# wardvdnb/Multimodal-SSL-AVMNIST

Hardware: NVIDIA B200
Metric: DINO train samples/sec (higher is better)
Workload: dtype bf16

## Files before the change

include/avmnist_b200.h:

```cpp
#ifndef AVMNIST_B200_H
#define AVMNIST_B200_H

#include <stdint.h>

#ifdef __cplusplus
extern "C" {
#endif

#define B200_E_ARG (-1)
#define B200_E_SHAPE (-2)
#define B200_E_SMEM (-3)

const char* b200_last_error(void);
int b200_abi_version(void);
int b200_device_sm_count(int device);
int b200_graph_node_counts(void* graph, int64_t* counts);

int b200_ema_flat(float* teacher, const float* student, int64_t n, float m, float one_minus_m, void* stream);
int b200_ema_multi(float* const* t_ptrs, const float* const* s_ptrs, const int64_t* offsets, int n_tensors,
                   int64_t total, float m, float one_minus_m, void* stream);

int b200_dino_loss_parts(int B);
int b200_dino_loss_fwd_bwd(const float* s, const float* t, const float* center, const float* t_colmean,
                           int Vs, int Vt, int B, int D, float tau_s, float tau_t, float grad_scale, int variant,
                           float* grad_s, float* part_loss, float* part_colsum, void* stream);
int b200_teacher_norm_colmean(const float* t, const float* center, int Vt, int B, int D, float* out, void* stream);

int b200_center_update(float* center, const float* part_colsum, const float* part_loss, int n_parts, int D,
                       int64_t n_rows, float m_c, float one_minus_mc, float* loss_out, float* colsum_out, void* stream);
int b200_center_apply(float* center, const float* colsum, int D, int64_t n_rows, float m_c, float one_minus_mc,
                      void* stream);

int64_t b200_loss_work_floats(int B);
int b200_mse_align_fwd_bwd(const float* a, const float* b, int B, int D, float grad_scale, float* grad_a,
                           float* grad_b, float* loss_out, float* work, void* stream);
int b200_ce_fwd_bwd(const float* logits, const int64_t* labels, int B, int C, float grad_scale, float* grad_logits,
                    float* loss_out, float* work, void* stream);
int64_t b200_infonce_work_floats(int B, int D);
int b200_infonce_fwd_bwd(const float* a, const float* b, int B, int D, float temperature, float grad_scale,
                         float* grad_a, float* grad_b, float* loss_out, float* work, void* stream);
int64_t b200_infonce_tc_work_floats(int B, int D);
int b200_infonce_fwd_bwd_tc(const float* a, const float* b, int B, int D, float temperature, float grad_scale, float* grad_a,
                            float* grad_b, float* loss_out, float* work, void* stream);
int64_t b200_ntxent_work_floats(int N, int D);
int b200_ntxent_fwd_bwd(const float* reps, int N, int D, float temperature, float grad_scale, float* grad, float* loss_out,
                        float* work, void* stream);
int b200_cosine_consistency_fwd_bwd(const float* emb, int V, int B, int D, float grad_scale, float* grad_emb,
                                    float* loss_out, float* work, void* stream);

#define B200_AUG_MAX_OPS 8
#define B200_AUG_GROUP_WORDS 28

int b200_aug_apply_image(const void* src, int src_u8, const int32_t* ops, float* out, void* out_quad8, int pad, int B,
                         int V, void* stream);
int b200_aug_apply_image_ex(const void* src, int src_u8, const int32_t* ops, const float* elastic_grid, uint64_t seed,
                            float* out, void* out_quad8, int pad, int B, int V, void* stream);
int b200_aug_apply_audio(const void* src, int src_u8, const int32_t* ops, const uint32_t* group_bits,
                         const float* noise, uint64_t seed, float* out, void* out_quad8, int pad, int B, int V,
                         void* stream);
int b200_aug_sample(const int32_t* spec, int B, int Vg, int Vl, uint64_t seed, uint64_t step, int32_t* img_ops,
                    int32_t* aud_ops, uint32_t* group_bits, void* stream);
int b200_aug_sample_dev(const int32_t* spec, int B, int Vg, int Vl, uint64_t seed, uint64_t step, const int64_t* step_dev,
                        int32_t* img_ops, int32_t* aud_ops, uint32_t* group_bits, void* stream);
int b200_aug_apply_audio_dev(const void* src, int src_u8, const int32_t* ops, const uint32_t* group_bits,
                             const float* noise, uint64_t seed, const int64_t* step_dev, float* out, void* out_quad8,
                             int pad, int B, int V, void* stream);

int b200_conv_supported(int Cin, int Cout, int H, int W, int K, int pad);
int b200_conv_fwd(const float* x, const float* w, const float* bias, float* z, double* stats, int N,
                  int n_per_view, int Cin, int Cout, int H, int W, int K, int pad, void* stream);
int b200_conv_bwd_data(const float* dz, const float* w, float* dx, int N, int Cin, int Cout, int H, int W, int K,
                       int pad, void* stream);
int b200_conv_tc_supported(int Cin, int Cout, int H, int W, int K, int pad);
int64_t b200_conv_tc_weight_bytes(int Cin, int Cout, int K);
int b200_conv_tc_prep_weights(const float* w, void* wprep, int Cin, int Cout, int K, int flip, void* stream);
int b200_conv_tc_prep_weights_multi(const int64_t* desc_dev, int n, void* stream);
int b200_conv_tc(const void* x_act8, const void* wprep, const float* bias, void* out, double* stats, int N,
                 int n_per_view, int Cin, int Cout, int H, int W, int K, int pad, int out_bf16, void* stream);
int b200_conv_tc_wgrad_variant(int tap);
int64_t b200_conv_tc_wgrad_work_floats(int N, int Cin, int Cout, int H, int W, int K, int pad);
int b200_conv_tc_wgrad(const void* x_act8, const void* dz_act8, float* dw, float* work, int N, int Cin, int Cout, int H,
                       int W, int K, int pad, void* stream);
int b200_pack_shift8(const float* x, void* out, int N, int H, int W, int pad, void* stream);
int b200_pack_quad8(const float* x, void* out, int N, int H, int W, int pad, void* stream);
int64_t b200_conv_tc_wgrad_l0_fused_work_floats(int N, int n_per_view, int Cout, int H, int W, int K, int pad);
int b200_conv_tc_wgrad_l0_fused(const void* x_quad8, const void* z8, const void* dp8, const float* scale, const float* shift,
                                const float* mean, const float* invstd, const double* sums, float* dw, double* dbsum,
                                float* work, int N, int n_per_view, int Cout, int H, int W, int K, int pad, void* stream);
int b200_conv_tc_pool_supported(int Cin, int Cout, int H, int W, int K, int pad);
int b200_conv_tc_pool(const void* x_act8, const void* wprep, const float* bias, const float* gamma, void* z_out, void* pool_out,
                      double* stats, int N, int n_per_view, int Cin, int Cout, int H, int W, int K, int pad, int z_fmt,
                      void* stream);
int b200_conv_tc_dgrad_bnstat_supported(int Cin, int Cout, int H, int W, int K, int pad);
int b200_conv_tc_dgrad_bnstat(const void* dz_act8, const void* wprep_flip, void* dx_act8, const void* p_act8, const float* gamma,
                              const float* beta, double* sums, int N, int n_per_view, int Cin, int Cout, int H, int W, int K,
                              int pad, void* stream);
int b200_bn_relu_apply8(const void* e8, const float* scale, const float* shift, void* out, int N, int n_per_view, int C, int HP,
                        int WP, int out_fmt, void* stream);
int b200_bn_relu_pool8_fwd(const void* z8, const float* scale, const float* shift, void* out, int N, int n_per_view,
                           int C, int H, int W, int z_f16, int out_fmt, void* stream);
int b200_bn_relu_pool8_bwd_reduce(const void* z8, const void* dp, const float* scale, const float* shift,
                                  const float* mean, const float* invstd, double* sums, int N, int n_per_view, int C,
                                  int H, int W, int z_f16, int dp_fmt, void* stream);
int b200_bn_relu_pool8_bwd_apply(const void* z8, const void* dp, const float* scale, const float* shift,
                                 const float* mean, const float* invstd, const double* sums, void* dz8, double* dbsum,
                                 int N, int n_per_view, int C, int H, int W, int z_f16, int dp_fmt, void* stream);
int b200_bn_pool8_bwd_reduce_p(const void* p, const void* dp, const float* gamma, const float* beta, double* sums, int N,
                               int n_per_view, int C, int HP, int WP, int p_fmt, int dp_fmt, void* stream);
int b200_bias_grad_finalize(const double* dbsum, float* db, int C, void* stream);
int b200_unpack_act8(const void* x8, float* out, int N, int C, int H, int W, void* stream);
int b200_pack_act8(const float* x, void* out, int N, int C, int H, int W, void* stream);
int64_t b200_conv_bwd_weight_work_floats(int N, int Cin, int Cout, int H, int W, int K, int pad);
int b200_conv_bwd_weight(const float* x, const float* dz, float* dw, float* db, float* work, int N, int Cin,
                         int Cout, int H, int W, int K, int pad, void* stream);

int b200_bn_finalize(const double* stats, const float* gamma, const float* beta, float* running_mean,
                     float* running_var, int64_t* num_batches_tracked, float* scale, float* shift, float* mean,
                     float* invstd, int n_views, int C, int64_t count, float momentum, float eps, int train,
                     void* stream);
int b200_bn_relu_pool_fwd(const float* z, const float* scale, const float* shift, float* out, int N,
                          int n_per_view, int C, int H, int W, void* stream);
int b200_bn_relu_pool_bwd_reduce(const float* z, const float* dout, const float* scale, const float* shift,
                                 const float* mean, const float* invstd, double* sums, int N, int n_per_view,
                                 int C, int H, int W, void* stream);
int b200_bn_relu_pool_bwd_apply(const float* z, const float* dout, const float* scale, const float* shift,
                                const float* mean, const float* invstd, const double* sums, float* dz, int N,
                                int n_per_view, int C, int H, int W, void* stream);
int b200_bn_param_grads(const double* sums, float* dgamma, float* dbeta, int n_views, int C, int accumulate,
                        void* stream);
int b200_avgpool_fwd(const float* x, float* out, int N, int C, int HW, void* stream);
int b200_avgpool_bwd(const float* dout, float* dx, int N, int C, int HW, void* stream);

int b200_linear_fwd(const float* x, int64_t ldx, const float* w, const float* bias, float* y, int64_t ldy, int M,
                    int N, int K, int act, const uint8_t* mask, float drop_p, void* stream);
int b200_linear_bwd_data(const float* dy, int64_t lddy, const float* w, float* dx, int64_t lddx, int M, int N,
                         int K, void* stream);
int64_t b200_linear_bwd_weight_work_floats(int M, int N, int K);
int b200_linear_bwd_weight(const float* dy, int64_t lddy, const float* x, int64_t ldx, float* dw, float* db, float* work,
                           int M, int N, int K, int accumulate, void* stream);
int b200_linear_fwd_tc(const float* x, int64_t ldx, const float* w, const float* bias, float* y, int64_t ldy, int M, int N,
                       int K, int act, const uint8_t* mask, float drop_p, void* stream);
int64_t b200_linear_bwd_data_tc_work_floats(int M, int N, int K);
int b200_linear_bwd_data_tc(const float* dy, int64_t lddy, const float* w, float* dx, int64_t lddx, float* work, int M, int N,
                            int K, void* stream);
int64_t b200_linear_bwd_weight_tc_work_floats(int M, int N, int K);
int b200_linear_bwd_weight_tc(const float* dy, int64_t lddy, const float* x, int64_t ldx, float* dw, float* db, float* work,
                              int M, int N, int K, int accumulate, void* stream);
int b200_act_bwd(float* dy, const float* y, const uint8_t* mask, float drop_p, int64_t n, void* stream);
int b200_colstats(const float* h, double* stats, int M, int C, void* stream);
int b200_bn1d_gelu_drop_fwd(const float* h, const float* scale, const float* shift, const uint8_t* mask,
                            float drop_p, float* g, int M, int C, void* stream);
int b200_bn1d_gelu_drop_bwd_reduce(const float* h, const float* dg, const float* scale, const float* shift,
                                   const float* mean, const float* invstd, const uint8_t* mask, float drop_p,
                                   double* sums, int M, int C, void* stream);
int b200_bn1d_gelu_drop_bwd_apply(const float* h, const float* dg, const float* scale, const float* shift,
                                  const float* mean, const float* invstd, const uint8_t* mask, float drop_p,
                                  const double* sums, float* dh, int M, int C, void* stream);
int b200_dropout_mask(uint8_t* mask, int64_t n, float p, uint64_t seed, uint64_t offset, void* stream);
int b200_dropout_mask_dev(uint8_t* mask, int64_t n, float p, uint64_t seed, uint64_t offset, const int64_t* step_dev,
                          void* stream);

int b200_adam_flat(float* param, const float* grad, float* exp_avg, float* exp_avg_sq, int64_t n, float lr,
                   float beta1, float beta2, float eps, float weight_decay, float bias_correction1,
                   float bias_correction2_sqrt, float grad_scale, void* stream);
int b200_adam_bias_dev(const int64_t* step_dev, double beta1, double beta2, float* bc_out, void* stream);
int b200_adam_flat_dev(float* param, const float* grad, float* exp_avg, float* exp_avg_sq, int64_t n, float lr,
                       float beta1, float beta2, float eps, float weight_decay, const float* bc_dev, float grad_scale,
                       void* stream);
int b200_counters_advance(int64_t* counters, int n, void* stream);
int b200_scale_flat(float* y, int64_t n, float alpha, void* stream);

int b200_knn_neg_half_sqnorm(const float* x, int64_t ldx, int N, int D, float* out, void* stream);
int b200_knn_topk_vote(const float* scores, int64_t lds, const int64_t* labels, int M, int N, int k, int n_classes,
                       int64_t* pred, int32_t* neighbours, void* stream);

int b200_gate_apply(const float* x, int64_t ldx, float* y, int64_t ldy, const float* gate, int M, int N, void* stream);
int64_t b200_gate_grad_work_floats(void);
int b200_gate_grad(const float* dy, int64_t lddy, const float* x, int64_t ldx, const float* gate, float* dgate, float* work, int M, int N,
                   int accumulate, void* stream);
int b200_softmax_rows(float* s, int64_t ld, int M, int N, float scale, void* stream);
int b200_softmax_rows_bwd(float* dp, int64_t lddp, const float* p, int64_t ldp, int M, int N, float scale, void* stream);
int b200_add2d(float* dst, int64_t ld_dst, const float* src, int64_t ld_src, int M, int N, void* stream);

int b200_dp_nccl_version(void);
int b200_dp_unique_id(char* id_out );
int b200_dp_init(const char* id , int rank, int world);
int b200_dp_world(void);
int b200_dp_rank(void);
int b200_dp_allreduce_grads(float* grad, int64_t n, void* stream);
int b200_dp_allreduce_center(float* colsum, int D, void* stream);
int b200_dp_destroy(void);

#ifdef __cplusplus
}
#endif
#endif
```

multimodal_ssl_avmnist_b200/contrastive.py:

```python
import math

import numpy as np
import torch

from . import dp
from . import ops
from .engine import F32, Arena, DinoStepEngine, _BN, _conv, _lin, _vec2, head_params

IMG_LAYERS = [("image_encoder.encoder.0", "image_encoder.encoder.1", 1, 32, 28, 3, 1), ("image_encoder.encoder.4", "image_encoder.encoder.5", 32, 64, 14, 3, 1),
              ("image_encoder.encoder.8", "image_encoder.encoder.9", 64, 128, 7, 3, 1)]
AUD_LAYERS = [("audio_encoder.encoder.0", "audio_encoder.encoder.1", 1, 32, 112, 3, 1), ("audio_encoder.encoder.4", "audio_encoder.encoder.5", 32, 64, 56, 3, 1),
              ("audio_encoder.encoder.8", "audio_encoder.encoder.9", 64, 128, 28, 3, 1), ("audio_encoder.encoder.12", "audio_encoder.encoder.13", 128, 256, 14, 3, 1)]
MODES = (("img", "img"), ("aud", "aud"), ("img", "aud"), ("aud", "img"))


def contrastive_params(O, P):
    img = []
    for i, (ci, co) in zip((0, 4, 8), ((1, 32), (32, 64), (64, 128))):
        img += _conv(f"image_encoder.encoder.{i}", co, ci, 3) + _vec2(f"image_encoder.encoder.{i + 1}", co)
    img += _lin("image_encoder.encoder.14", 512, 128) + _lin("image_encoder.projection.0", O, 512)
    img += [("image_projection_head." + n, s) for n, s in head_params(O, P)]
    aud = []
    for i, (ci, co) in zip((0, 4, 8, 12), ((1, 32), (32, 64), (64, 128), (128, 256))):
        aud += _conv(f"audio_encoder.encoder.{i}", co, ci, 3) + _vec2(f"audio_encoder.encoder.{i + 1}", co)
    aud += _lin("audio_encoder.encoder.18", O, 256)
    aud += [("audio_projection_head." + n, s) for n, s in head_params(O, P)]
    return img, aud


class ContrastiveStepEngine(DinoStepEngine):
    def __init__(self, kind="infonce", output_dim=256, projection_dim=256, learning_rate=1e-4, temperature=0.07, seed=0, device=None,
                 precision="bf16", fused_pool=False, process_group=None, data_parallel=None, mode_seed=0):
        if not torch.cuda.is_available():
            raise ops._lib.B200Error("ContrastiveStepEngine needs a CUDA device: the hot path has no CPU fallback")
        ops._lib.load()
        assert kind in ("infonce", "simclr") and precision in ("bf16", "fp32")
        self.device = torch.device(device if device is not None else f"cuda:{torch.cuda.current_device()}")
        self.kind, self.mode, self.precision = kind, "default", precision
        self.lin_tc = precision == "bf16"
        self.multi, self.mix = False, None
        self.O, self.P = output_dim, projection_dim
        self.lr, self.weight_decay, self.temperature = learning_rate, 0.0, temperature
        self.seed, self.rng_step = seed, 0
        self.pg = process_group
        self.world = dp.world_size(process_group) if (data_parallel is None or data_parallel) else 1
        self.comm, self._comm_stream = None, None
        self._ctr = self._bc = self._graph = None
        self.img_layers, self.aud_layers = IMG_LAYERS, AUD_LAYERS
        img, aud = contrastive_params(self.O, self.P)
        self.student = Arena([("enc." + n, s) for n, s in img + aud], self.device)
        self.branch_range = {"img": self.student.range_of(["enc." + n for n, _ in img]), "aud": self.student.range_of(["enc." + n for n, _ in aud])}
        self.step_counts = {"img": 0, "aud": 0}
        self.grad = torch.zeros_like(self.student.flat)
        self.exp_avg, self.exp_avg_sq = torch.zeros_like(self.student.flat), torch.zeros_like(self.student.flat)
        self.S, self.G = self.student.views(), self.student.views(self.grad)
        self.bn_s = {}
        for conv, bn, ci, co, hw, k, pad in IMG_LAYERS + AUD_LAYERS:
            self.bn_s["enc." + bn] = _BN(co, self.device)
        for m in ("image", "audio"):
            self.bn_s[f"enc.{m}_projection_head.mlp.1"] = _BN(512, self.device)
        self.tc = {}
        for mod, layers in (("img", IMG_LAYERS), ("aud", AUD_LAYERS)):
            self.tc[mod] = [precision == "bf16" and ops.conv_tc_supported(ci, co, hw, hw, k, pad) and
                            (ci == 1 or ops.conv_tc_supported(co, ci, hw + 2 * pad - k + 1, hw + 2 * pad - k + 1, k, k - 1 - pad))
                            for (conv, bn, ci, co, hw, k, pad) in layers]
        self.fused_pool = bool(fused_pool)
        self.pool = {"s": {mod: [self.fused_pool and bool(self.tc[mod][li]) and ops.conv_tc_pool_supported(ci, co, hw, hw, k, pad) and ci == 1 and hw >= 112
                                 for li, (conv, bn, ci, co, hw, k, pad) in enumerate(layers)] for mod, layers in (("img", IMG_LAYERS), ("aud", AUD_LAYERS))}}
        self.pool["t"] = self.pool["s"]
        self.fused_bnstat = False
        self.bnstat = {mod: [False] * len(layers) for mod, layers in (("img", IMG_LAYERS), ("aud", AUD_LAYERS))}
        self._tcw, self._prep_desc = {}, {}
        for mod, layers in (("img", IMG_LAYERS), ("aud", AUD_LAYERS)):
            for li, (conv, bn, ci, co, hw, k, pad) in enumerate(layers):
                if self.tc[mod][li]:
                    self._tcw[("s", mod, li)] = torch.empty(ops.conv_tc_weight_bytes(ci, co, k), dtype=torch.uint8, device=self.device)
                    if ci > 1:
                        self._tcw[("flip", mod, li)] = torch.empty(ops.conv_tc_weight_bytes(co, ci, k), dtype=torch.uint8, device=self.device)
        self.overlap_teacher = True
        self.stream_priorities, self._main_stream = False, None
        self._side_stream = torch.cuda.Stream(device=self.device)
        self._lin_wg_stream = torch.cuda.Stream(device=self.device)
        self._lin_wg_pending = False
        self._wgrad_streams = {m: torch.cuda.Stream(device=self.device) for m in ("img", "aud")}
        self._eval_wrole = "s"
        self._ws = {}
        self._mode_rng = torch.Generator().manual_seed(mode_seed)
        if self.world > 1:
            self.comm = dp.AbiComm.get(process_group)
            self._comm_stream = torch.cuda.Stream(device=self.device)
        self._comm_pending = False
        self._init_parameters()

    def _init_parameters(self):
        g = torch.Generator(device="cpu").manual_seed(self.seed)
        bn_bases = set(self.bn_s)
        bounds = {}
        for name, shape in self.student.spec:
            v = self.student.view(name)
            base = name.rsplit(".", 1)[0]
            if base in bn_bases:
                v.fill_(1.0 if name.endswith(".weight") else 0.0)
            else:
                if len(shape) > 1:
                    bounds[base] = 1.0 / math.sqrt(int(np.prod(shape[1:])))
                v.copy_(((torch.rand(shape, generator=g) * 2 - 1) * bounds[base]).to(self.device))

    def load_named(self, params):
        for m, d in params.items():
            for k, v in d.items():
                self.S[f"enc.{m}.{k}"].copy_(v.to(self.device))

    def sync_teacher(self):
        pass

    def _dino_only(self, *a, **k):
        raise ops._lib.B200Error("this entry point belongs to the DINO step engine; the contrastive engine offers forward_backward / "
                                 "optimizer_step / train_step_views / train_step / capture_train_step / graph_step")

    forward_pass = dino_loss_pass = aux_loss_pass = backward_pass = update_teacher = train_step_host = encode_features = begin_probe = _dino_only
    augment = augment_with_params = prefetch_augment = allreduce_gradients = graph_node_counts = _dino_only

    def _workspace(self, B):
        if B in self._ws:
            return self._ws[B]
        dev, BF = self.device, torch.bfloat16

        def e(*shape, dtype=F32):
            return torch.empty(*shape, dtype=dtype, device=dev)

        w = {"B": B}
        zarena = torch.zeros(1 << 16, dtype=torch.float64, device=dev)
        zoff = [0]

        def zalloc(*shape):
            n = int(math.prod(shape))
            o = zoff[0]
            zoff[0] = o + (n + 1) // 2 * 2
            if zoff[0] > zarena.numel():
                raise ops._lib.B200Error("zero arena too small")
            return zarena[o:o + n].view(*shape)

        w["zarena"] = zarena
        N = 2 * B
        w["x_img"], w["x_aud"] = e(N, 1, 28, 28), e(N, 1, 112, 112)
        for mod, layers in (("img", IMG_LAYERS), ("aud", AUD_LAYERS)):
            sc = dict(wg=0, z=0, p=0, z8=0)
            for li, (conv, bn, ci, co, hw, k, pad) in enumerate(layers):
                ho = hw + 2 * pad - k + 1
                tc = self.tc[mod][li]
                next_tc = li + 1 < len(layers) and self.tc[mod][li + 1]
                if tc and ci == 1:
                    w[f"{mod}.xs8"] = e(N, hw, ops.quad8_width(hw, pad), 8, dtype=BF)
                if tc and self.pool["s"][mod][li]:
                    w[f"s.{mod}.e{li}"] = e(N, co // 8, ho // 2, ho // 2, 8, dtype=torch.float16)
                w[f"s.{mod}.z{li}"] = e(N, co // 8, ho, ho, 8, dtype=torch.float16) if tc else e(N, co, ho, ho)
                if next_tc:
                    w[f"s.{mod}.p8{li}"] = e(N, co // 8, ho // 2, ho // 2, 8, dtype=BF)
                if not next_tc or not tc:
                    w[f"s.{mod}.p{li}"] = e(N, co, ho // 2, ho // 2)
                w[f"s.{mod}.stats{li}"] = zalloc(2, co, 2)
                w[f"s.{mod}.sums{li}"] = zalloc(2, co, 2)
                for nm in ("scale", "shift", "mean", "invstd"):
                    w[f"s.{mod}.{nm}{li}"] = e(2, co)
                if tc:
                    sc["wg"] = max(sc["wg"], ops.conv_tc_wgrad_work_floats(N, ci, co, hw, hw, k, pad))
                    if ci == 1:
                        sc["wg"] = max(sc["wg"], ops.conv_tc_wgrad_l0_fused_work_floats(N, B, co, hw, hw, k, pad))
                    else:
                        sc["z8"] = max(sc["z8"], N * co * ho * ho)
                else:
                    sc["wg"] = max(sc["wg"], ops.conv_bwd_weight_work_floats(N, ci, co, hw, hw, k, pad))
                    sc["z"] = max(sc["z"], N * co * ho * ho)
                sc["p"] = max(sc["p"], N * co * (ho // 2) * (ho // 2), N * ci * hw * hw if li > 0 else 0)
            w[f"{mod}.dz"] = e(max(sc["z"], 4))
            w[f"{mod}.dz8"] = e(max(sc["z8"], 8), dtype=BF)
            w[f"{mod}.dz8b"] = e(max(sc["z8"], 8), dtype=BF)
            w[f"{mod}.dbsum"] = zalloc(8, 256)
            w[f"{mod}.dp_a"], w[f"{mod}.dp_b"] = e(sc["p"]), e(sc["p"])
            w[f"{mod}.wg_work"], w[f"{mod}.wg_work_b"] = e(max(sc["wg"], 4)), e(max(sc["wg"], 4))
        O, P = self.O, self.P
        w["img.gap"], w["img.e14"], w["aud.gap"] = e(N, 128), e(N, 512), e(N, 256)
        w["d.img.gap"], w["d.img.e14"], w["d.aud.gap"] = e(N, 128), e(N, 512), e(N, 256)
        for mod in ("img", "aud"):
            w[f"{mod}.feat"], w[f"d.{mod}.feat"] = e(N, O), e(N, O)
            w[f"{mod}.hh"], w[f"{mod}.g"], w[f"{mod}.d.hh"], w[f"{mod}.d.g"] = e(N, 512), e(N, 512), e(N, 512), e(N, 512)
            w[f"{mod}.hstats"], w[f"{mod}.hsums"] = zalloc(2, 512, 2), zalloc(2, 512, 2)
            for nm in ("hscale", "hshift", "hmean", "hinvstd"):
                w[f"{mod}.{nm}"] = e(2, 512)
        w["reps"], w["d.reps"] = e(N, P), e(N, P)
        w["loss"] = torch.zeros(4, device=dev)
        w["ntxent_work"] = e(ops.ntxent_work_floats(N, P))
        w["infonce_work"] = e(ops.infonce_work_floats(B, P, tc=self.lin_tc))
        self._ws[B] = w
        return w

    def _combo(self, w, mod, calls):
        key = ("combo", mod, calls)
        if key in w:
            return w[key]
        B = w["B"]
        N = calls * B
        c = {"B": B, "zarena": w["zarena"], "packed": False}
        for k, v in w.items():
            if not isinstance(k, str) or not isinstance(v, torch.Tensor):
                continue
            if k.startswith(f"s.{mod}.") and k.split(".")[2].rstrip("0123456789") in ("stats", "sums", "scale", "shift", "mean", "invstd"):
                c[k] = v[:calls]
            elif k.startswith(f"s.{mod}.") or k == f"{mod}.xs8":
                c[k] = v[:N]
            elif k.startswith(f"{mod}."):
                c[k] = v
        w[key] = c
        return c

    def _branch_fwd(self, w, mod, x, calls):
        B, S = w["B"], self.S
        N = calls * B
        c = self._combo(w, mod, calls)
        layers = IMG_LAYERS if mod == "img" else AUD_LAYERS
        hw = layers[0][4]
        xin = w[f"x_{mod}"][:N]
        xin.copy_(x.reshape(N, 1, hw, hw))
        if self.tc[mod][0]:
# ... 231 lines not shown
```

multimodal_ssl_avmnist_b200/csrc/conv_tc.cu:

```cuda
#include <cuda_bf16.h>

#include "common.cuh"
#include "umma.cuh"

namespace b200 {

int encode_tmap_bf16_4d(CUtensorMap* out, const void* base, const uint64_t dims[4], const uint64_t strides_bytes[3],
                        const uint32_t box[4]) {
    typedef CUresult (*EncodeFn)(CUtensorMap*, CUtensorMapDataType, cuuint32_t, void*, const cuuint64_t*, const cuuint64_t*,
                                 const cuuint32_t*, const cuuint32_t*, CUtensorMapInterleave, CUtensorMapSwizzle,
                                 CUtensorMapL2promotion, CUtensorMapFloatOOBfill);
    static EncodeFn fn = nullptr;
    if (!fn) {
        void* p = nullptr;
        cudaDriverEntryPointQueryResult q;
        cudaError_t e = cudaGetDriverEntryPoint("cuTensorMapEncodeTiled", &p, cudaEnableDefault, &q);
        if (e != cudaSuccess || q != cudaDriverEntryPointSuccess || !p) {
            set_error("cuTensorMapEncodeTiled entry point not available (%d)", (int)e);
            return -30;
        }
        fn = (EncodeFn)p;
    }
    cuuint64_t d[4] = {dims[0], dims[1], dims[2], dims[3]};
    cuuint64_t s[3] = {strides_bytes[0], strides_bytes[1], strides_bytes[2]};
    cuuint32_t b[4] = {box[0], box[1], box[2], box[3]};
    cuuint32_t es[4] = {1, 1, 1, 1};
    CUresult r = fn(out, CU_TENSOR_MAP_DATA_TYPE_BFLOAT16, 4, const_cast<void*>(base), d, s, b, es, CU_TENSOR_MAP_INTERLEAVE_NONE,
                    CU_TENSOR_MAP_SWIZZLE_NONE, CU_TENSOR_MAP_L2_PROMOTION_L2_128B, CU_TENSOR_MAP_FLOAT_OOB_FILL_NONE);
    if (r != CUDA_SUCCESS) {
        set_error("cuTensorMapEncodeTiled failed (%d)", (int)r);
        return -31;
    }
    return 0;
}

namespace {

using namespace umma;

constexpr int round_up(int a, int b) { return (a + b - 1) / b * b; }
constexpr int SMEM_EST(int nmma, int npad, int slots, int slot_bytes, int tail) { return round_up(nmma * npad * 32, 128) + slots * slot_bytes + tail + 256 + npad * 4; }
constexpr int nbuf_for(int npadl, int ctas) {
    int n = (npadl <= 32 ? 8 : 4) / (ctas > 2 ? 2 : 1);
    while (n > 1 && n * npadl * ctas > 512) n /= 2;
    return n;
}
constexpr int pow2_cols(int c) { return c <= 32 ? 32 : c <= 64 ? 64 : c <= 128 ? 128 : c <= 256 ? 256 : 512; }

__host__ __device__ constexpr int xph_for(int cin, int cout, int ks) {
    return (ks == 5 && ((cin == 8 && cout == 16) || (cin == 16 && cout == 8))) ? 4
         : (ks == 5 && ((cin == 16 && cout == 32) || (cin == 32 && cout == 16))) ? 2
         : (ks == 3 && ((cin == 32 && cout == 64) || (cin == 64 && cout == 32))) ? 2 : 1;
}

struct TMaps {
    CUtensorMap m[4];
};

constexpr int nbuf_chunked(int tiles, int npadl, int ctas) {
    int m = 512 / (ctas * npadl * tiles);
    while (m > 1 && m * tiles > 8) --m;
    return (m < 1 ? 1 : m) * tiles;
}

template <int CIN_, int COUT_, int NPAD_, int HIN_, int WIN_, int KS_, int PAD_, int BANDS_, int SLOTS_, int CTAS_ = 1, int NSPLIT_ = 1, int KCH_ = 1>
struct TcCfg {
    static constexpr int NSPLIT = NSPLIT_;
    static constexpr int KCH = KCH_;
    static constexpr int XPH = CIN_ == 1 ? 4 : xph_for(CIN_, COUT_, KS_);
    static constexpr int XPL = CIN_ == 1 ? 1 : XPH;
    __host__ __device__ static constexpr int col_phase(int col) { return (col / 8) % XPH; }
    __host__ __device__ static constexpr int col_channel(int col) { return (col / 8) / XPH * 8 + col % 8; }
    static constexpr int NPADL = XPH == 1 ? NPAD_ / NSPLIT_ : round_up(XPH * COUT_, 16), COUTL = COUT_ / NSPLIT_;
    static_assert(NSPLIT_ == 1 || (XPH == 1 && COUT_ == NPAD_ && NPADL % 16 == 0), "N split needs C_out == NPAD and 16-channel slices");
    static constexpr int CIN = CIN_, COUT = COUT_, NPAD = NPAD_, HIN = HIN_, WIN = WIN_, KS = KS_, PAD = PAD_, BANDS = BANDS_, SLOTS = SLOTS_;
    static constexpr int CTAS = CTAS_;
    static constexpr bool L0 = (CIN == 1);
    static constexpr int P = L0 ? 1 : CIN / 8;
    static constexpr int WP = WIN + 2 * PAD;
    static constexpr int HO = HIN + 2 * PAD - KS + 1, WO = WP - KS + 1;
    static constexpr int HB = HO / BANDS;
    static constexpr int HPB = HB + KS - 1;
    static constexpr int KWX = KS + XPH - 1;
    static constexpr int WQ = (WP + XPH - 1) / XPH;
    static constexpr int WOQ = WO / XPH;
    static constexpr int Q = (HB - 1) * WQ + WOQ;
    static constexpr int TILES = (Q + 127) / 128;
    static constexpr int PLANE_BYTES = HPB * WQ * 16;
    static constexpr int PC = P / KCH;
    static constexpr int PHASE_BYTES = round_up(PC * PLANE_BYTES, 128);
    static constexpr int SLOT_BYTES = round_up(XPL * PHASE_BYTES, 128);
    static constexpr int NJ = (KWX + 1) / 2;
    static constexpr int PH = P / 2;
    static constexpr int PHC = PC / 2;
    static constexpr int NMMA = L0 ? (KS + 1) / 2 : (CIN == 8) ? KS * NJ : KS * KWX * PH;
    static constexpr int W_BYTES = round_up(NMMA * NPADL * 32, 128);
    static constexpr int MAXPIX = TILES * 128 + (L0 ? KS : KS - 1) * WQ + (KWX - 1) / XPH + 2;
    static constexpr int TAIL = round_up((MAXPIX > HPB * WQ ? (MAXPIX - HPB * WQ) : 0) * 16, 128) + 128;
    static_assert(XPH == 1 || (WO % XPH == 0 && WIN % XPH == 0 && XPH <= 4 && (CIN != 8 || (XPH % 2 == 0 && KWX % 2 == 0))), "x phases");
    static_assert(!L0 || KWX <= 8, "first layer: all taps of all phases must lie inside one 8-pixel unit");
    static constexpr int IMG_BYTES = SLOTS * SLOT_BYTES + TAIL;
    static constexpr int BAR_OFF = W_BYTES + IMG_BYTES;
    static constexpr bool POOL_OK = (CIN_ == 1 || COUT_ > CIN_) && NSPLIT_ == 1 && HO % 2 == 0 && HB % 2 == 0 && WO % 2 == 0 && XPH % 2 == 0;
    static constexpr bool BSTAT_OK = CIN_ > COUT_ && NSPLIT_ == 1;
    static constexpr int POOL_R = 128 / WQ + 3;
    static constexpr int OCTL = COUTL / 8;
    static constexpr int POOL_ROW_UNITS = (WO / 2) * OCTL;
    static constexpr int POOL_BYTES = POOL_OK ? POOL_R * POOL_ROW_UNITS * 16 : 0;
    static constexpr int SIGN_OFF = BAR_OFF + 256 + NPADL * 4;
    static constexpr int POOL_OFF = round_up(SIGN_OFF + NPADL * 2, 16);
    static constexpr int SMEM = POOL_OFF + POOL_BYTES;
    static constexpr int SMEM_NOPOOL = SIGN_OFF + NPADL * 4;
    static constexpr int NBUF = KCH > 1 ? nbuf_chunked(TILES, NPADL, CTAS) : nbuf_for(NPADL, CTAS);
    static_assert(KCH == 1 || (CIN >= 16 && P % KCH == 0 && PC % 2 == 0 && NBUF % TILES == 0 && NBUF * NPADL * CTAS <= 512), "K chunking");
    static constexpr int TMEM_COLS = pow2_cols(NBUF * NPADL);
    static constexpr int ISS = CTAS >= 3 ? 1 : (CTAS == 2 ? 2 : 4);
    static constexpr int THREADS = 32 * (1 + ISS + 4);
    static_assert(TILES % ISS == 0 || NBUF % TILES == 0, "a TMEM stage must always be filled by the same issuer");
    static_assert(KCH > 1 || NBUF % ISS == 0, "a TMEM stage must always be filled by the same issuer");
    static_assert(TMEM_COLS * CTAS <= 512, "TMEM columns per SM");
    static_assert((SMEM_EST(NMMA, NPADL, SLOTS, SLOT_BYTES, TAIL) + POOL_BYTES + NPADL * 2 + 16 + 1024) * CTAS <= 227 * 1024, "shared memory per SM");
    static_assert(2 * SLOTS + 2 * NBUF <= 24, "barrier area");
    static_assert(CIN == 1 || (CIN % 8 == 0 && (CIN == 8 || CIN % 16 == 0)), "C_in must be 1, 8 or a multiple of 16");
    static_assert(NPAD % 16 == 0 && NPAD >= 16 && NPADL <= 128 && COUT <= NPAD && COUT % 8 == 0, "N tile");
    static_assert(HO % BANDS == 0, "bands must divide the output height");
    static_assert(SMEM <= 227 * 1024, "shared memory budget");
    static_assert(XPL * PHASE_BYTES < (1 << 18) && PLANE_BYTES % 16 == 0, "descriptor range");
};

__device__ __forceinline__ void ld_global_nc_256(const uint4* p, uint4& a, uint4& b) {
    asm volatile("ld.global.nc.v8.b32 {%0, %1, %2, %3, %4, %5, %6, %7}, [%8];"
                 : "=r"(a.x), "=r"(a.y), "=r"(a.z), "=r"(a.w), "=r"(b.x), "=r"(b.y), "=r"(b.z), "=r"(b.w)
                 : "l"(p));
}
__device__ __forceinline__ uint32_t hmax2_u32(uint32_t a, uint32_t b) {
    uint32_t d;
    asm("max.f16x2 %0, %1, %2;" : "=r"(d) : "r"(a), "r"(b));
    return d;
}
template <class C>
__device__ __forceinline__ int pool_unit(int h, int xq) {
    if constexpr (C::XPH % 2 == 0) {
        const int col0 = h * 16;
        if (col0 >= C::XPH * C::COUTL) return -1;
        const int ph0 = C::col_phase(col0), oct0 = C::col_channel(col0) / 8;
        return ((xq * C::XPH + ph0) >> 1) * C::OCTL + oct0;
    } else {
        const int oct = h;
        if (oct * 8 >= C::COUTL) return -1;
        return (xq >> 1) * C::OCTL + oct;
    }
}

template <class C, bool POOL, bool BSTAT = false>
__global__ void __launch_bounds__(C::THREADS, C::CTAS)
conv_tc_kernel(const __grid_constant__ TMaps tmaps, const uint4* __restrict__ wprep, const float* __restrict__ bias,
               void* __restrict__ out, double* __restrict__ stats, int n_per_view, int out_bf16,
               uint4* __restrict__ pool_out, const float* __restrict__ gamma, const float* __restrict__ beta2 = nullptr) {
    extern __shared__ __align__(1024) uint8_t smem[];
    uint8_t* w_s = smem;
    uint8_t* img_s = smem + C::W_BYTES;
    uint64_t* bars = reinterpret_cast<uint64_t*>(smem + C::BAR_OFF);
    uint32_t* tmem_slot = reinterpret_cast<uint32_t*>(smem + C::BAR_OFF + 200);
    float* bias_s = reinterpret_cast<float*>(smem + C::BAR_OFF + 256);
    uint32_t* sign_s = reinterpret_cast<uint32_t*>(smem + C::SIGN_OFF);
    float* ig_s = reinterpret_cast<float*>(smem + C::SIGN_OFF);
    uint4* stash = reinterpret_cast<uint4*>(smem + C::POOL_OFF);

    const int warp = threadIdx.x >> 5, lane = threadIdx.x & 31;
    const int view = blockIdx.y, G = gridDim.x, g = blockIdx.x;
    const long items = (long)n_per_view * C::BANDS;
    const int i0 = (int)(items * g / G), i1 = (int)(items * (g + 1) / G);

    const uint32_t bar0 = smem_u32(bars);
    auto full_bar = [&](int s) { return bar0 + 8u * s; };
    auto empty_bar = [&](int s) { return bar0 + 8u * (C::SLOTS + s); };
    auto tfull_bar = [&](int b) { return bar0 + 8u * (2 * C::SLOTS + b); };
    auto tempty_bar = [&](int b) { return bar0 + 8u * (2 * C::SLOTS + C::NBUF + b); };

    {
        const uint4* src = wprep;
        uint4* dst = reinterpret_cast<uint4*>(w_s);
        constexpr int NGL = C::NPADL / 8, NG = NGL * C::NSPLIT;
        for (int i = threadIdx.x; i < C::NMMA * 2 * NGL * 8; i += blockDim.x) {
            const int q = i & 7, gl = (i >> 3) % NGL, mc = (i >> 3) / NGL;
            dst[i] = src[(mc * NG + blockIdx.z * NGL + gl) * 8 + q];
        }
        uint4* z = reinterpret_cast<uint4*>(img_s);
        for (int i = threadIdx.x; i < C::IMG_BYTES / 16; i += blockDim.x) z[i] = make_uint4(0, 0, 0, 0);
        for (int i = threadIdx.x; i < C::NPADL; i += blockDim.x)
            bias_s[i] = (bias != nullptr && i < C::XPH * C::COUTL) ? bias[blockIdx.z * C::COUTL + C::col_channel(i)] : 0.f;
        if constexpr (BSTAT) {
            for (int i = threadIdx.x; i < C::NPADL; i += blockDim.x) {
                const bool real = i < C::XPH * C::COUTL;
                const float gm = real ? gamma[blockIdx.z * C::COUTL + C::col_channel(i)] : 0.f;
                ig_s[i] = gm != 0.f ? 1.0f / gm : 0.f;
                bias_s[i] = real ? beta2[blockIdx.z * C::COUTL + C::col_channel(i)] : 0.f;
            }
        }
        if constexpr (POOL) {
            for (int i = threadIdx.x; i < C::NPADL / 2; i += blockDim.x) {
                uint32_t m = 0;
#pragma unroll
                for (int h = 0; h < 2; ++h) {
                    const int col = 2 * i + h;
                    if (gamma != nullptr && col < C::XPH * C::COUTL && gamma[blockIdx.z * C::COUTL + C::col_channel(col)] < 0.f) m |= 0x8000u << (16 * h);
                }
                sign_s[i] = m;
            }
        }
        fence_proxy_async_smem();
    }
    if (warp == 0 && lane == 0) {
        for (int r = 0; r < C::XPL; ++r) prefetch_tmap(&tmaps.m[r]);
        for (int s = 0; s < C::SLOTS; ++s) {
            mbar_init(full_bar(s), 1);
            mbar_init(empty_bar(s), C::ISS);
        }
        for (int b = 0; b < C::NBUF; ++b) {
            mbar_init(tfull_bar(b), 1);
            mbar_init(tempty_bar(b), 4);
        }
        fence_mbar_init();
    }
    if (warp == 1) tmem_alloc<C::TMEM_COLS>(smem_u32(tmem_slot));
    tc_fence_before_sync();
    __syncthreads();
    tc_fence_after_sync();
    const uint32_t tmem_base = *tmem_slot;
    const uint32_t img_addr = smem_u32(img_s), w_addr = smem_u32(w_s);

    if (warp == 0) {
        if (lane == 0) {
            for (int i = i0; i < i1; ++i) {
                const int n = view * n_per_view + i / C::BANDS, band = i % C::BANDS;
#pragma unroll 1
                for (int c = 0; c < C::KCH; ++c) {
                    const int k = (i - i0) * C::KCH + c, slot = k % C::SLOTS, use = k / C::SLOTS;
                    mbar_wait(empty_bar(slot), (use & 1) ^ 1);
                    mbar_expect_tx(full_bar(slot), C::XPL * C::PC * C::PLANE_BYTES);
#pragma unroll
                    for (int rp = 0; rp < C::XPL; ++rp) {
                        constexpr int X = C::XPH;
                        const int r = ((rp - C::PAD) % X + X) % X, a = (rp - C::PAD - r) / X;
                        tma_load_4d(img_addr + slot * C::SLOT_BYTES + rp * C::PHASE_BYTES, &tmaps.m[r], full_bar(slot), 0, C::L0 ? 0 : a,
                                    band * C::HB - C::PAD, n * C::P + c * C::PC);
                    }
                }
            }
        }
    } else if (warp <= C::ISS) {
        if (lane == 0) {
            constexpr uint32_t idesc = idesc_bf16(C::NPADL);
            for (int i = i0; i < i1; ++i) {
#pragma unroll 1
              for (int c = 0; c < C::KCH; ++c) {
                const int k = (i - i0) * C::KCH + c, slot = k % C::SLOTS, use = k / C::SLOTS;
                mbar_wait(full_bar(slot), use & 1);
                tc_fence_after_sync();
                const uint32_t slot_addr = img_addr + slot * C::SLOT_BYTES;
                for (int t = warp - 1; t < C::TILES; t += C::ISS) {
                    const uint32_t tcount = (uint32_t)(i - i0) * C::TILES + t;
                    const uint32_t buf = tcount % C::NBUF, u = tcount / C::NBUF;
                    if (c == 0) {
                        mbar_wait(tempty_bar(buf), (u & 1) ^ 1);
                        tc_fence_after_sync();
                    }
                    const uint32_t d = tmem_base + buf * C::NPADL;
                    const uint32_t a0 = slot_addr + t * 2048;
                    int idx = 0;
                    if constexpr (C::L0) {
#pragma unroll
                        for (int j = 0; j < C::NMMA; ++j, ++idx) {
                            const uint64_t ad = smem_desc(a0 + (2 * j * C::WQ) * 16, C::WQ * 16, 128);
                            const uint64_t bd = smem_desc(w_addr + idx * C::NPADL * 32, C::NPADL * 16, 128);
                            mma_bf16(d, ad, bd, idesc, idx > 0);
                        }
                    } else {
#pragma unroll
                    for (int kh = 0; kh < C::KS; ++kh) {
                        if constexpr (C::CIN == 8) {
#pragma unroll
                            for (int j = 0; j < C::NJ; ++j, ++idx) {
                                const uint64_t ad = smem_desc(a0 + ((2 * j) % C::XPH) * C::PHASE_BYTES + (kh * C::WQ + (2 * j) / C::XPH) * 16,
                                                              C::XPH == 1 ? 16 : C::PHASE_BYTES, 128);
                                const uint64_t bd = smem_desc(w_addr + idx * C::NPADL * 32, C::NPADL * 16, 128);
                                mma_bf16(d, ad, bd, idesc, idx > 0);
                            }
                        } else {
#pragma unroll
                            for (int kw = 0; kw < C::KWX; ++kw) {
#pragma unroll
                                for (int pp = 0; pp < C::PHC; ++pp, ++idx) {
                                    const int widx = (kh * C::KWX + kw) * C::PH + c * C::PHC + pp;
                                    const uint64_t ad = smem_desc(a0 + (kw % C::XPH) * C::PHASE_BYTES + (kh * C::WQ + kw / C::XPH) * 16 +
                                                                      pp * 2 * C::PLANE_BYTES, C::PLANE_BYTES, 128);
                                    const uint64_t bd = smem_desc(w_addr + widx * C::NPADL * 32, C::NPADL * 16, 128);
                                    mma_bf16(d, ad, bd, idesc, (c > 0 || idx > 0) ? 1u : 0u);
                                }
                            }
                        }
                    }
                    }
                    if (c == C::KCH - 1) mma_commit(tfull_bar(buf));
                }
                mma_commit(empty_bar(slot));
              }
            }
        }
    } else {
        const int quad = warp & 3, row = quad * 32 + lane;
        float s1[C::COUTL], s2[C::COUTL];
#pragma unroll
        for (int c = 0; c < C::COUTL; ++c) s1[c] = s2[c] = 0.f;
        const int co0 = blockIdx.z * C::COUTL;
        const bool do_stats = BSTAT ? (stats != nullptr) : ((bias != nullptr) && (stats != nullptr));
        constexpr int NCH = C::NPADL / 16;
        constexpr int NHP = POOL ? (C::XPH % 2 == 0 ? NCH : 2 * NCH) : 1;
        uint32_t tcount = 0;
        for (int i = i0; i < i1; ++i) {
            const int n = view * n_per_view + i / C::BANDS, band = i % C::BANDS;
            for (int t = 0; t < C::TILES; ++t, ++tcount) {
                [[maybe_unused]] uint4 hp[NHP];
                const uint32_t buf = tcount % C::NBUF, u = tcount / C::NBUF;
                const int q = t * 128 + row;
                const int y = q / C::WQ, xq = q - y * C::WQ;
                const bool valid = (y < C::HB) && (xq < C::WOQ);
                const int yy = band * C::HB + y;
                [[maybe_unused]] uint4 ppre[BSTAT ? NCH : 1][2];
                if constexpr (BSTAT) {
#pragma unroll
                    for (int cc = 0; cc < NCH; ++cc) {
                        const int col0 = cc * 16;
                        ppre[cc][0] = ppre[cc][1] = make_uint4(0, 0, 0, 0);
                        if (valid && col0 < C::XPH * C::COUTL) {
                            const int ph0 = C::col_phase(col0), oct0 = C::col_channel(col0) / 8;
                            const uint4* pin = pool_out;
                            if constexpr (C::XPH % 2 == 0) {
                                ld_global_nc_256(pin + (((long)n * (C::COUT / 8) + co0 / 8 + oct0) * C::HO + yy) * C::WO + xq * C::XPH + ph0, ppre[cc][0],
                                                 ppre[cc][1]);
                            } else {
                                ppre[cc][0] = __ldg(pin + (((long)n * (C::COUT / 8) + co0 / 8 + oct0) * C::HO + yy) * C::WO + xq);
                                if ((oct0 + 1) * 8 < C::COUTL)
                                    ppre[cc][1] = __ldg(pin + (((long)n * (C::COUT / 8) + co0 / 8 + oct0 + 1) * C::HO + yy) * C::WO + xq);
                            }
                        }
                    }
                }
                mbar_wait(tfull_bar(buf), u & 1);
                tc_fence_after_sync();
                const uint32_t taddr = tmem_base + ((uint32_t)(quad * 32) << 16) + buf * C::NPADL;
#pragma unroll
                for (int cc = 0; cc < C::NPADL / 16; ++cc) {
                    uint32_t v[16];
                    tmem_ld16(taddr + cc * 16, v);
                    tmem_ld_wait();
                    if (cc == C::NPADL / 16 - 1) {
                        tc_fence_before_sync();
                        __syncwarp();
                        if (lane == 0) mbar_arrive(tempty_bar(buf));
                    }
                    float f[16];
#pragma unroll
                    for (int j = 0; j < 16; ++j) {
                        const int col = cc * 16 + j, ch = C::col_channel(col);
                        if constexpr (BSTAT) {
                            f[j] = __uint_as_float(v[j]);
                        } else {
                            f[j] = __uint_as_float(v[j]) + bias_s[col];
                            if (col < C::XPH * C::COUTL && valid) {
                                s1[ch] += f[j];
                                s2[ch] += f[j] * f[j];
                            }
                        }
                    }
                    if constexpr (BSTAT) {
                        const int col0 = cc * 16;
                        if (valid && col0 < C::XPH * C::COUTL) {
                            const uint4 pa = ppre[cc][0], pb = ppre[cc][1];
                            const uint32_t pw[8] = {pa.x, pa.y, pa.z, pa.w, pb.x, pb.y, pb.z, pb.w};
#pragma unroll
                            for (int j = 0; j < 16; ++j) {
                                const int col = col0 + j, ch = C::col_channel(col);
                                const float pv = __uint_as_float((j & 1) ? (pw[j >> 1] & 0xFFFF0000u) : (pw[j >> 1] << 16));
                                const float gr = __bfloat162float(__float2bfloat16_rn(f[j]));
                                if (col < C::XPH * C::COUTL && pv > 0.f) {
                                    s1[ch] += gr;
                                    s2[ch] += gr * ((pv - bias_s[col]) * ig_s[col]);
                                }
                            }
                        }
                    }
                    if constexpr (POOL) {
                        {
                            uint4 a, b;
                            a.x = pack_f16(f[0], f[1]); a.y = pack_f16(f[2], f[3]); a.z = pack_f16(f[4], f[5]); a.w = pack_f16(f[6], f[7]);
                            b.x = pack_f16(f[8], f[9]); b.y = pack_f16(f[10], f[11]); b.z = pack_f16(f[12], f[13]); b.w = pack_f16(f[14], f[15]);
                            const uint4 ma = *reinterpret_cast<const uint4*>(sign_s + cc * 8), mb = *reinterpret_cast<const uint4*>(sign_s + cc * 8 + 4);
                            a.x ^= ma.x; a.y ^= ma.y; a.z ^= ma.z; a.w ^= ma.w;
                            b.x ^= mb.x; b.y ^= mb.y; b.z ^= mb.z; b.w ^= mb.w;
                            if constexpr (C::XPH % 2 == 0) {
                                hp[cc].x = hmax2_u32(a.x, b.x); hp[cc].y = hmax2_u32(a.y, b.y); hp[cc].z = hmax2_u32(a.z, b.z); hp[cc].w = hmax2_u32(a.w, b.w);
                            } else {
                                hp[2 * cc].x = hmax2_u32(a.x, __shfl_xor_sync(0xffffffffu, a.x, 1)); hp[2 * cc].y = hmax2_u32(a.y, __shfl_xor_sync(0xffffffffu, a.y, 1));
                                hp[2 * cc].z = hmax2_u32(a.z, __shfl_xor_sync(0xffffffffu, a.z, 1)); hp[2 * cc].w = hmax2_u32(a.w, __shfl_xor_sync(0xffffffffu, a.w, 1));
                                hp[2 * cc + 1].x = hmax2_u32(b.x, __shfl_xor_sync(0xffffffffu, b.x, 1)); hp[2 * cc + 1].y = hmax2_u32(b.y, __shfl_xor_sync(0xffffffffu, b.y, 1));
                                hp[2 * cc + 1].z = hmax2_u32(b.z, __shfl_xor_sync(0xffffffffu, b.z, 1)); hp[2 * cc + 1].w = hmax2_u32(b.w, __shfl_xor_sync(0xffffffffu, b.w, 1));
                            }
                        }
                    }
                    if (valid && (!POOL || out != nullptr)) {
                        if (out_bf16) {
                            uint4 pk[2];
#pragma unroll
                            for (int o = 0; o < 2; ++o) {
                                if (out_bf16 == 2) {
                                    pk[o].x = pack_f16(f[o * 8 + 0], f[o * 8 + 1]);
                                    pk[o].y = pack_f16(f[o * 8 + 2], f[o * 8 + 3]);
                                    pk[o].z = pack_f16(f[o * 8 + 4], f[o * 8 + 5]);
                                    pk[o].w = pack_f16(f[o * 8 + 6], f[o * 8 + 7]);
                                } else {
                                    pk[o].x = pack_bf16(f[o * 8 + 0], f[o * 8 + 1]);
                                    pk[o].y = pack_bf16(f[o * 8 + 2], f[o * 8 + 3]);
                                    pk[o].z = pack_bf16(f[o * 8 + 4], f[o * 8 + 5]);
                                    pk[o].w = pack_bf16(f[o * 8 + 6], f[o * 8 + 7]);
                                }
                            }
                            const int col0 = cc * 16, ph0 = C::col_phase(col0), oct0 = C::col_channel(col0) / 8;
                            if constexpr (C::XPH % 2 == 0) {
                                if (col0 < C::XPH * C::COUTL) {
                                    uint4* dst = reinterpret_cast<uint4*>(out) + (((long)n * (C::COUT / 8) + co0 / 8 + oct0) * C::HO + yy) * C::WO +
                                                 xq * C::XPH + ph0;
                                    st_global_256(dst, pk[0], pk[1]);
                                }
                            } else {
#pragma unroll
                                for (int o = 0; o < 2; ++o) {
                                    const int oct = oct0 + o;
                                    if (oct * 8 < C::COUTL) {
                                        uint4* dst = reinterpret_cast<uint4*>(out) + (((long)n * (C::COUT / 8) + co0 / 8 + oct) * C::HO + yy) * C::WO + xq;
                                        *dst = pk[o];
                                    }
                                }
                            }
                        } else {
                            float* dst = reinterpret_cast<float*>(out) + (((long)n * C::COUT + co0) * C::HO + yy) * C::WO + xq * C::XPH;
#pragma unroll
                            for (int j = 0; j < 16; ++j) {
                                const int col = cc * 16 + j, ph = C::col_phase(col), ch = C::col_channel(col);
                                if (col < C::XPH * C::COUTL) dst[(long)ch * C::HO * C::WO + ph] = f[j];
                            }
                        }
                    }
                }
                if constexpr (POOL) {
                    {
                        const int slot = (int)(((long)(i - i0) * (C::HB / 2) + (y >> 1)) % C::POOL_R);
                        const bool own = valid && (C::XPH % 2 == 0 || (xq & 1) == 0);
                        uint4* srow = stash + slot * C::POOL_ROW_UNITS;
                        if (own && (y & 1) == 0) {
#pragma unroll
                            for (int h = 0; h < NHP; ++h) {
                                const int u = pool_unit<C>(h, xq);
                                if (u >= 0) srow[u] = hp[h];
                            }
                        }
                        asm volatile("bar.sync 2, 128;" ::: "memory");
                        if (own && (y & 1) == 1) {
                            const int ypg = (band * C::HB + y) >> 1;
                            uint4 ev[NHP];
#pragma unroll
                            for (int h = 0; h < NHP; ++h) {
                                const int u = pool_unit<C>(h, xq);
                                if (u >= 0) {
                                    const uint4 up = srow[u];
                                    const int col0 = (C::XPH % 2 == 0 ? h : h / 2) * 16 + (C::XPH % 2 == 0 ? 0 : (h & 1) * 8);
                                    const uint4 m = *reinterpret_cast<const uint4*>(sign_s + col0 / 2);
                                    ev[h].x = hmax2_u32(hp[h].x, up.x) ^ m.x; ev[h].y = hmax2_u32(hp[h].y, up.y) ^ m.y;
                                    ev[h].z = hmax2_u32(hp[h].z, up.z) ^ m.z; ev[h].w = hmax2_u32(hp[h].w, up.w) ^ m.w;
                                }
                            }
                            const long plane = (long)(C::HO / 2) * (C::WO / 2);
                            uint4* erow = pool_out + ((long)n * (C::COUT / 8) + co0 / 8) * plane + (long)ypg * (C::WO / 2);
                            if constexpr (C::XPH == 4) {
#pragma unroll
                                for (int h = 0; h + 1 < NHP; h += 2) {
                                    const int u = pool_unit<C>(h, xq);
                                    if (u >= 0) {
                                        const int xp = u / C::OCTL, oct = u - xp * C::OCTL;
                                        st_global_256(erow + oct * plane + xp, ev[h], ev[h + 1]);
                                    }
                                }
                            } else {
#pragma unroll
                                for (int h = 0; h < NHP; ++h) {
                                    const int u = pool_unit<C>(h, xq);
                                    if (u >= 0) {
                                        const int xp = u / C::OCTL, oct = u - xp * C::OCTL;
                                        erow[oct * plane + xp] = ev[h];
                                    }
                                }
                            }
                        }
                    }
                }
            }
        }
        if (do_stats) {
#pragma unroll
            for (int c = 0; c < C::COUTL; ++c) {
                const double a = warp_sum((double)s1[c]), b = warp_sum((double)s2[c]);
                if (lane == 0) {
                    atomicAdd(&stats[((long)view * C::COUT + co0 + c) * 2 + 0], a);
                    atomicAdd(&stats[((long)view * C::COUT + co0 + c) * 2 + 1], b);
                }
            }
        }
    }
    tc_fence_before_sync();
    __syncthreads();
    if (warp == 1) {
        tc_fence_after_sync();
        tmem_dealloc<C::TMEM_COLS>(tmem_base);
    }
}

__device__ __forceinline__ void conv_tc_prep_element(const float* __restrict__ w, __nv_bfloat16* __restrict__ out, int CIN, int COUT, int NPAD,
                                                     int KS, int XPH, int flip, int e) {
    const int k8 = e & 7, r = (e >> 3) & 7, NG = NPAD / 8;
    const int ng = (e >> 6) % NG, c = (e / (64 * NG)) & 1, m = e / (128 * NG);
    const int ph = ng % XPH, co = ng / XPH * 8 + r;
    const int KWX = KS + XPH - 1;
    int kh, kw, ci;
    if (CIN == 1) {
        kh = 2 * m + c;
        kw = k8 - ph;
        ci = 0;
        float v1 = 0.f;
        if (kh < KS && kw >= 0 && kw < KS && co < COUT) v1 = w[(co * KS + kh) * KS + kw];
        out[e] = __float2bfloat16_rn(v1);
        return;
    } else if (CIN == 8) {
        const int NJ = (KWX + 1) / 2;
        kh = m / NJ;
        kw = 2 * (m % NJ) + c - ph;
        ci = k8;
    } else {
        const int PH = CIN / 16;
        kh = m / (KWX * PH);
        kw = (m / PH) % KWX - ph;
        ci = (2 * (m % PH) + c) * 8 + k8;
    }
    float v = 0.f;
    if (kw >= 0 && kw < KS && co < COUT) {
        v = flip ? w[((ci * COUT + co) * KS + (KS - 1 - kh)) * KS + (KS - 1 - kw)] : w[((co * CIN + ci) * KS + kh) * KS + kw];
    }
    out[e] = __float2bfloat16_rn(v);
}

__global__ void conv_tc_prep_weights_kernel(const float* __restrict__ w, __nv_bfloat16* __restrict__ out, int CIN, int COUT, int NPAD,
                                            int KS, int XPH, int flip, int total) {
    const int e = blockIdx.x * blockDim.x + threadIdx.x;
    if (e < total) conv_tc_prep_element(w, out, CIN, COUT, NPAD, KS, XPH, flip, e);
}

__host__ __device__ inline void conv_tc_weight_geometry(int Cin, int Cout, int K, int* xph, int* npad, int* total) {
    const int x = Cin == 1 ? 4 : xph_for(Cin, Cout, K), kwx = K + x - 1;
    const int np = (x * Cout + 15) / 16 * 16;
    const int nmma = (Cin == 1) ? (K + 1) / 2 : (Cin == 8) ? K * ((kwx + 1) / 2) : K * kwx * (Cin / 16);
    *xph = x;
    *npad = np;
    *total = nmma * np * 16;
}

__global__ void conv_tc_prep_weights_multi_kernel(const long long* __restrict__ desc) {
    const long long* d = desc + 6 * blockIdx.y;
    const int Cin = (int)d[2], Cout = (int)d[3], K = (int)d[4], flip = (int)d[5];
    int xph, npad, total;
    conv_tc_weight_geometry(Cin, Cout, K, &xph, &npad, &total);
    const float* w = reinterpret_cast<const float*>(d[0]);
    __nv_bfloat16* out = reinterpret_cast<__nv_bfloat16*>(d[1]);
    for (int e = blockIdx.x * blockDim.x + threadIdx.x; e < total; e += gridDim.x * blockDim.x)
        conv_tc_prep_element(w, out, Cin, Cout, npad, K, xph, flip, e);
}

__global__ void pack_act8_kernel(const float* __restrict__ x, uint4* __restrict__ out, long n_units, int C, int HW) {
    const long i = (long)blockIdx.x * blockDim.x + threadIdx.x;
    if (i >= n_units) return;
    const int pix = (int)(i % HW);
    const long no = i / HW;
    const int oct = (int)(no % (C / 8));
    const long n = no / (C / 8);
    const float* s = x + ((n * C + oct * 8) * (long)HW) + pix;
    uint4 pk;
    pk.x = pack_bf16(s[0], s[(long)HW]);
    pk.y = pack_bf16(s[2L * HW], s[3L * HW]);
    pk.z = pack_bf16(s[4L * HW], s[5L * HW]);
    pk.w = pack_bf16(s[6L * HW], s[7L * HW]);
    out[i] = pk;
}

__global__ void pack_shift8_kernel(const float* __restrict__ x, uint4* __restrict__ out, long n_units, int W, int pad) {
    const long i = (long)blockIdx.x * blockDim.x + threadIdx.x;
    if (i >= n_units) return;
    const int WT = W + pad;
    const int xs = (int)(i % WT);
    const long row = i / WT;
    const float* r = x + row * W;
    float f[8];
#pragma unroll
    for (int c = 0; c < 8; ++c) {
        const int xc = xs - pad + c;
        f[c] = (xc >= 0 && xc < W) ? __ldg(r + xc) : 0.f;
    }
    out[i] = make_uint4(pack_bf16(f[0], f[1]), pack_bf16(f[2], f[3]), pack_bf16(f[4], f[5]), pack_bf16(f[6], f[7]));
}

__global__ void pack_quad8_kernel(const float* __restrict__ x, uint4* __restrict__ out, long n_units, int W, int WQ, int pad) {
    const long i = (long)blockIdx.x * blockDim.x + threadIdx.x;
    if (i >= n_units) return;
    const int xq = (int)(i % WQ);
    const long row = i / WQ;
    const float* r = x + row * W;
    float f[8];
#pragma unroll
    for (int c = 0; c < 8; ++c) {
        const int xc = 4 * xq - pad + c;
        f[c] = (xc >= 0 && xc < W) ? __ldg(r + xc) : 0.f;
    }
    out[i] = make_uint4(pack_bf16(f[0], f[1]), pack_bf16(f[2], f[3]), pack_bf16(f[4], f[5]), pack_bf16(f[6], f[7]));
}

template <class C>
int launch_conv_tc(const void* x, const void* wprep, const float* bias, void* out, double* stats, int N, int n_per_view, int out_bf16,
                   cudaStream_t st, void* pool_out = nullptr, const float* gamma = nullptr, const float* beta2 = nullptr) {
    if (pool_out != nullptr && beta2 == nullptr && !C::POOL_OK) {
        set_error("conv_tc: this geometry has no fused max-pool epilogue");
        return -5;
    }
    static bool configured = false;
    if (!configured) {
        cudaError_t e = cudaFuncSetAttribute(conv_tc_kernel<C, false>, cudaFuncAttributeMaxDynamicSharedMemorySize, C::SMEM_NOPOOL);
        if (e == cudaSuccess && C::POOL_OK) e = cudaFuncSetAttribute(conv_tc_kernel<C, C::POOL_OK>, cudaFuncAttributeMaxDynamicSharedMemorySize, C::SMEM);
        if (e == cudaSuccess && C::BSTAT_OK)
            e = cudaFuncSetAttribute(conv_tc_kernel<C, false, C::BSTAT_OK>, cudaFuncAttributeMaxDynamicSharedMemorySize, C::SMEM_NOPOOL);
        if (e != cudaSuccess) {
            set_error("conv_tc: cannot set %d bytes of shared memory: %s", C::SMEM, cudaGetErrorString(e));
            return (int)e;
        }
        configured = true;
    }
    TMaps tm;
    constexpr uint64_t WT = C::L0 ? C::WQ : C::WIN;
    for (int r = 0; r < C::XPL; ++r) {
        const uint64_t dims[4] = {8, WT / C::XPL, (uint64_t)C::HIN, (uint64_t)N * C::P};
        const uint64_t strides[3] = {16 * (uint64_t)C::XPL, WT * 16, WT * C::HIN * 16};
        const uint32_t box[4] = {8, (uint32_t)C::WQ, (uint32_t)C::HPB, (uint32_t)C::PC};
        int rc = encode_tmap_bf16_4d(&tm.m[r], reinterpret_cast<const uint8_t*>(x) + 16 * r, dims, strides, box);
        if (rc) return rc;
    }
    for (int r = C::XPL; r < 4; ++r) tm.m[r] = tm.m[0];
    const int views = N / n_per_view;
    int G = sm_count() * C::CTAS / (views * C::NSPLIT);
    if (G < 1) G = 1;
    const long items = (long)n_per_view * C::BANDS;
    if (G > items) G = (int)items;
    if (beta2 != nullptr) {
        if (!C::BSTAT_OK) {
            set_error("conv_tc: this geometry has no fused BatchNorm-backward statistics");
            return -5;
        }
        conv_tc_kernel<C, false, C::BSTAT_OK><<<dim3(G, views, C::NSPLIT), C::THREADS, C::SMEM_NOPOOL, st>>>(
            tm, reinterpret_cast<const uint4*>(wprep), nullptr, out, stats, n_per_view, out_bf16, reinterpret_cast<uint4*>(pool_out), gamma, beta2);
    } else if (pool_out != nullptr)
        conv_tc_kernel<C, C::POOL_OK><<<dim3(G, views, C::NSPLIT), C::THREADS, C::SMEM, st>>>(tm, reinterpret_cast<const uint4*>(wprep), bias, out, stats,
                                                                                              n_per_view, out_bf16, reinterpret_cast<uint4*>(pool_out), gamma);
    else
        conv_tc_kernel<C, false><<<dim3(G, views, C::NSPLIT), C::THREADS, C::SMEM_NOPOOL, st>>>(tm, reinterpret_cast<const uint4*>(wprep), bias, out, stats,
                                                                                                n_per_view, out_bf16, nullptr, nullptr);
    return launch_status("conv_tc_kernel");
}

constexpr int hbz_for(int hb, int wp) {
    int h = hb;
    while ((h * wp) % 16) ++h;
    return h;
}

template <int CIN_, int COUT_, int HIN_, int WIN_, int KS_, int PAD_, int BANDS_, int SLOTS_, int PSPLIT_, int CTAS_ = 1, int NSPLIT_ = 1>
struct TcWgCfg {
    static constexpr int NSPLIT = NSPLIT_, COUTL = COUT_ / NSPLIT_;
    static constexpr int CTAS = CTAS_;
    static constexpr int CIN = CIN_, COUT = COUT_, HIN = HIN_, WIN = WIN_, KS = KS_, PAD = PAD_, BANDS = BANDS_, SLOTS = SLOTS_, PSPLIT = PSPLIT_;
    static constexpr bool L0 = (CIN == 1);
    static constexpr int P_IN = L0 ? 1 : CIN / 8, P_OUT = COUT / 8, P_OUTL = COUTL / 8, PI = P_IN / PSPLIT;
    static constexpr int WP = WIN + 2 * PAD;
    static constexpr int HO = HIN + 2 * PAD - KS + 1, WO = WP - KS + 1;
    static constexpr int HB = HO / BANDS, HPB = HB + KS - 1;
    static constexpr int HBZ = hbz_for(HB, WP);
    static constexpr int KSTEPS = HBZ * WP / 16;
    static constexpr int PLANE_X = HPB * WP * 16, PLANE_Z = HBZ * WP * 16;
    static constexpr int X_BYTES = round_up(PI * PLANE_X, 128), Z_BYTES = round_up(P_OUTL * PLANE_Z, 128);
    static constexpr int SLOT_BYTES = X_BYTES + Z_BYTES;
    static constexpr int NACC = L0 ? 1 : KS * PI;
    static constexpr int TMEM_COLS = pow2_cols(NACC * COUTL);
    static constexpr int ONES_OFF = SLOTS * SLOT_BYTES;
    static constexpr int BAR_OFF = ONES_OFF;
    static constexpr int SMEM = BAR_OFF + 256;
    static constexpr int DW = COUT * CIN * KS * KS;
    static constexpr int PART = DW;
    static_assert(P_IN % PSPLIT == 0 && HO % BANDS == 0, "splits");
    static_assert(BANDS == 1 || HBZ == HB, "row bands need HB*WP to be a multiple of 16");
    static constexpr int ISS = (L0 || NACC < 4 || CTAS >= 3) ? 1 : (NACC <= 6 ? NACC : 4);
    static constexpr int THREADS = 32 * (1 + ISS + 4);
    static_assert(NACC * COUTL <= 512 && TMEM_COLS * CTAS <= 512 && COUTL % 8 == 0, "TMEM columns");
    static_assert((SMEM + 1024) * CTAS <= 227 * 1024, "shared memory per SM");
    static_assert(KS <= 8 && COUT % 8 == 0 && COUT >= 8 && COUT <= 256, "shape");
    static_assert((KSTEPS * 16 + (L0 ? 7 : KS - 1) * WP + 8 - HPB * WP) * 16 <= Z_BYTES, "x overrun must stay inside the slot");
    static_assert(SMEM <= 227 * 1024, "shared memory budget");
};

template <class C>
__global__ void __launch_bounds__(C::THREADS, C::CTAS)
conv_tc_wgrad_kernel(const __grid_constant__ CUtensorMap tmap_x, const __grid_constant__ CUtensorMap tmap_z, float* __restrict__ work, int N) {
    extern __shared__ __align__(1024) uint8_t smem[];
    uint64_t* bars = reinterpret_cast<uint64_t*>(smem + C::BAR_OFF);
    uint32_t* tmem_slot = reinterpret_cast<uint32_t*>(smem + C::BAR_OFF + 192);
    const int warp = threadIdx.x >> 5, lane = threadIdx.x & 31;
    const int G = gridDim.x, g = blockIdx.x, split = blockIdx.z % C::PSPLIT, ns = blockIdx.z / C::PSPLIT;
    const long items = (long)N * C::BANDS;
    const int i0 = (int)(items * g / G), i1 = (int)(items * (g + 1) / G);
    const uint32_t bar0 = smem_u32(bars);
    auto full_bar = [&](int s) { return bar0 + 8u * s; };
    auto empty_bar = [&](int s) { return bar0 + 8u * (C::SLOTS + s); };
    const uint32_t done_bar = bar0 + 8u * (2 * C::SLOTS);
    {
        uint4* z = reinterpret_cast<uint4*>(smem);
        for (int i = threadIdx.x; i < C::ONES_OFF / 16; i += blockDim.x) z[i] = make_uint4(0, 0, 0, 0);
        fence_proxy_async_smem();
    }
    if (warp == 0 && lane == 0) {
        prefetch_tmap(&tmap_x);
        prefetch_tmap(&tmap_z);
        for (int s = 0; s < C::SLOTS; ++s) {
            mbar_init(full_bar(s), 1);
            mbar_init(empty_bar(s), C::ISS);
        }
        mbar_init(done_bar, C::ISS);
        fence_mbar_init();
    }
    if (warp == 1) tmem_alloc<C::TMEM_COLS>(smem_u32(tmem_slot));
    tc_fence_before_sync();
    __syncthreads();
    tc_fence_after_sync();
    const uint32_t tmem_base = *tmem_slot;
    const uint32_t smem0 = smem_u32(smem);

    if (warp == 0) {
        if (lane == 0) {
            for (int i = i0; i < i1; ++i) {
                const int k = i - i0, slot = k % C::SLOTS, use = k / C::SLOTS;
                mbar_wait(empty_bar(slot), (use & 1) ^ 1);
                mbar_expect_tx(full_bar(slot), C::PI * C::PLANE_X + C::P_OUTL * C::PLANE_Z);
                const int n = i / C::BANDS, band = i % C::BANDS;
                const uint32_t sa = smem0 + slot * C::SLOT_BYTES;
                tma_load_4d(sa, &tmap_x, full_bar(slot), 0, C::L0 ? 0 : -C::PAD, band * C::HB - C::PAD, n * C::P_IN + split * C::PI);
                tma_load_4d(sa + C::X_BYTES, &tmap_z, full_bar(slot), 0, 0, band * C::HB, n * C::P_OUT + ns * C::P_OUTL);
            }
        }
    } else if (warp <= C::ISS) {
        if (lane == 0) {
            constexpr uint32_t idesc = idesc_bf16(C::COUTL, true, true, 64);
            for (int i = i0; i < i1; ++i) {
                const int k = i - i0, slot = k % C::SLOTS, use = k / C::SLOTS;
                mbar_wait(full_bar(slot), use & 1);
                tc_fence_after_sync();
                const uint32_t xa = smem0 + slot * C::SLOT_BYTES, za = xa + C::X_BYTES;
                for (int ks = 0; ks < C::KSTEPS; ++ks) {
                    const uint32_t acc = (i > i0 || ks > 0) ? 1u : 0u;
                    const uint64_t bd = smem_desc(za + ks * 256, 128, C::PLANE_Z);
                    if constexpr (C::L0) {
                        const uint64_t ad = smem_desc(xa + ks * 256, 128, C::WP * 16);
                        mma_bf16(tmem_base, ad, bd, idesc, acc);
                    } else {
#pragma unroll
                        for (int kh = 0; kh < C::KS; ++kh) {
#pragma unroll
                            for (int pl = 0; pl < C::PI; ++pl) {
                                if ((kh * C::PI + pl) % C::ISS != warp - 1) continue;
                                const uint64_t ad = smem_desc(xa + pl * C::PLANE_X + (ks * 16 + kh * C::WP) * 16, 128, 16);
                                mma_bf16(tmem_base + (kh * C::PI + pl) * C::COUTL, ad, bd, idesc, acc);
                            }
                        }
                    }
                }
                mma_commit(empty_bar(slot));
            }
            mma_commit(done_bar);
        }
    } else {
        const int quad = warp & 3;
        const int m = quad * 16 + (lane & 15), j = m >> 3, ci8 = m & 7;
        const bool rowok = (lane < 16) && (j < C::KS);
        float* part = work + (long)g * C::PART;
        if (i1 > i0) {
            mbar_wait(done_bar, 0);
            tc_fence_after_sync();
        }
#pragma unroll 1
        for (int a = 0; a < C::NACC; ++a) {
            const int kh = a / C::PI, pl = a % C::PI;
#pragma unroll
            for (int cc = 0; cc < (C::COUTL + 15) / 16; ++cc) {
                uint32_t v[16];
// ... 858 lines not shown
    WGP_RUN(WgA1) WGP_RUN(WgA2)
#undef WGP_RUN
#define WGT_RUN(CFG) if (g_wgrad_tap && Cin == CFG::CIN && Cout == CFG::COUT && H == CFG::HIN && W == CFG::WIN && K == CFG::KS && pad == CFG::PAD) \
        return launch_conv_tc_wgrad_tap<CFG>(x, dz, dw, work, N, st, need);
    WGT_RUN(TapB1) WGT_RUN(TapB2) WGT_RUN(TapB3) WGT_RUN(TapS1) WGT_RUN(TapS2)
#undef WGT_RUN
    WG_RUN(WgA3) WG_RUN(WgI1) WG_RUN(WgS1) WG_RUN(WgA0) WG_RUN(WgI0) WG_RUN(WgS0) WG_RUN(WgS2) WG_RUN(WgB0) WG_RUN(WgB1) WG_RUN(WgB2) WG_RUN(WgB3)
#undef WG_RUN
    set_error("conv_tc_wgrad: unsupported geometry Cin=%d Cout=%d H=%d W=%d K=%d pad=%d", Cin, Cout, H, W, K, pad);
    return -4;
}

using WgF_A0 = L0FCfg<8, 112, 112, 5, 2, 7, 2, 2>;
using WgF_I0 = L0FCfg<32, 28, 28, 5, 2, 1, 2, 1>;
using WgF_S0 = L0FCfg<32, 28, 28, 3, 1, 1, 2, 1>;
using WgF_B0 = L0FCfg<32, 112, 112, 3, 1, 7, 1, 2, 2>;

static int wgrad_l0_dispatch(const void* x, const void* z, const void* dp, const float* scale, const float* shift, const float* mean,
                             const float* invstd, const double* sums, float* dw, double* dbsum, float* work, int N, int n_per_view, int Cout,
                             int H, int W, int K, int pad, cudaStream_t st, int64_t* need) {
#define WF_RUN(CFG) if (Cout == CFG::COUT && H == CFG::HIN && W == CFG::WIN && K == CFG::KS && pad == CFG::PAD) \
        return launch_conv_tc_wgrad_l0_fused<CFG>(x, z, dp, scale, shift, mean, invstd, sums, dw, dbsum, work, N, n_per_view, st, need);
    WF_RUN(WgF_A0) WF_RUN(WgF_I0) WF_RUN(WgF_S0) WF_RUN(WgF_B0)
#undef WF_RUN
    set_error("conv_tc_wgrad_l0_fused: unsupported geometry Cout=%d H=%d W=%d K=%d pad=%d", Cout, H, W, K, pad);
    return -4;
}

int64_t b200_conv_tc_wgrad_l0_fused_work_floats(int N, int n_per_view, int Cout, int H, int W, int K, int pad) {
    int64_t need = 0;
    if (N <= 0 || n_per_view <= 0 || N % n_per_view) return -1;
    int rc = wgrad_l0_dispatch(nullptr, nullptr, nullptr, nullptr, nullptr, nullptr, nullptr, nullptr, nullptr, nullptr, nullptr, N, n_per_view, Cout, H, W,
                               K, pad, nullptr, &need);
    return rc ? -1 : need;
}

int b200_conv_tc_wgrad_l0_fused(const void* x_quad8, const void* z8, const void* dp8, const float* scale, const float* shift,
                                const float* mean, const float* invstd, const double* sums, float* dw, double* dbsum, float* work, int N,
                                int n_per_view, int Cout, int H, int W, int K, int pad, void* stream) {
    B200_REQUIRE(x_quad8 && z8 && dp8 && scale && shift && mean && invstd && sums && dw && work, -1, "conv_tc_wgrad_l0_fused: null pointer");
    B200_REQUIRE(N > 0 && n_per_view > 0 && N % n_per_view == 0, -2, "conv_tc_wgrad_l0_fused: N=%d must be a multiple of n_per_view=%d", N, n_per_view);
    B200_REQUIRE(((reinterpret_cast<uintptr_t>(x_quad8) | reinterpret_cast<uintptr_t>(z8) | reinterpret_cast<uintptr_t>(dp8) |
                   reinterpret_cast<uintptr_t>(work)) & 15) == 0, -3, "conv_tc_wgrad_l0_fused: pointers must be 16-byte aligned");
    return wgrad_l0_dispatch(x_quad8, z8, dp8, scale, shift, mean, invstd, sums, dw, dbsum, work, N, n_per_view, Cout, H, W, K, pad,
                             as_stream(stream), nullptr);
}

int b200_conv_tc_wgrad_variant(int tap) {
    const int old = g_wgrad_tap;
    if (tap == 0 || tap == 1) g_wgrad_tap = tap;
    return old;
}

int64_t b200_conv_tc_wgrad_work_floats(int N, int Cin, int Cout, int H, int W, int K, int pad) {
    int64_t need = 0;
    int rc = wgrad_tc_dispatch(nullptr, nullptr, nullptr, nullptr, N, Cin, Cout, H, W, K, pad, nullptr, &need);
    return rc ? -1 : need;
}

int b200_conv_tc_wgrad(const void* x_act8, const void* dz_act8, float* dw, float* work, int N, int Cin, int Cout, int H, int W,
                       int K, int pad, void* stream) {
    B200_REQUIRE(x_act8 && dz_act8 && dw && work, -1, "conv_tc_wgrad: null pointer");
    B200_REQUIRE(N > 0, -2, "conv_tc_wgrad: N must be positive");
    B200_REQUIRE(((uintptr_t)x_act8 & 15) == 0 && ((uintptr_t)dz_act8 & 15) == 0, -3, "conv_tc_wgrad: pointers must be 16-byte aligned");
    return wgrad_tc_dispatch(x_act8, dz_act8, dw, work, N, Cin, Cout, H, W, K, pad, as_stream(stream), nullptr);
}

int b200_pack_quad8(const float* x, void* out, int N, int H, int W, int pad, void* stream) {
    B200_REQUIRE(x && out && N > 0 && H > 0 && W > 0 && pad >= 0, -1, "pack_quad8: bad arguments");
    const int WQ = (W + 2 * pad + 3) / 4;
    const long units = (long)N * H * WQ;
    pack_quad8_kernel<<<(unsigned)((units + 255) / 256), 256, 0, as_stream(stream)>>>(x, reinterpret_cast<uint4*>(out), units, W, WQ, pad);
    return launch_status("pack_quad8_kernel");
}

int b200_pack_shift8(const float* x, void* out, int N, int H, int W, int pad, void* stream) {
    B200_REQUIRE(x && out, -1, "pack_shift8: null pointer");
    B200_REQUIRE(N > 0 && H > 0 && W > 0 && pad >= 0, -2, "pack_shift8: bad shape");
    const long px = (long)N * H * (W + pad);
    pack_shift8_kernel<<<(unsigned)((px + 255) / 256), 256, 0, as_stream(stream)>>>(x, reinterpret_cast<uint4*>(out), px, W, pad);
    return launch_status("pack_shift8_kernel");
}

int b200_pack_act8(const float* x, void* out, int N, int C, int H, int W, void* stream) {
    B200_REQUIRE(x && out, -1, "pack_act8: null pointer");
    B200_REQUIRE(C % 8 == 0 && N > 0, -2, "pack_act8: C must be a multiple of 8");
    const long units = (long)N * (C / 8) * H * W;
    pack_act8_kernel<<<(unsigned)((units + 255) / 256), 256, 0, as_stream(stream)>>>(x, reinterpret_cast<uint4*>(out), units, C, H * W);
    return launch_status("pack_act8_kernel");
}

int b200_conv_tc(const void* x_act8, const void* wprep, const float* bias, void* out, double* stats, int N, int n_per_view, int Cin, int Cout,
                 int H, int W, int K, int pad, int out_bf16, void* stream) {
    B200_REQUIRE(x_act8 && wprep && out, -1, "conv_tc: null pointer");
    B200_REQUIRE(N > 0 && n_per_view > 0 && N % n_per_view == 0, -2, "conv_tc: N=%d must be a multiple of n_per_view=%d", N, n_per_view);
    B200_REQUIRE(((uintptr_t)x_act8 & 15) == 0 && ((uintptr_t)wprep & 15) == 0 && ((uintptr_t)out & 15) == 0, -3, "conv_tc: pointers must be 16-byte aligned");
    cudaStream_t st = as_stream(stream);
#define TC_RUN(CFG) if (Cin == CFG::CIN && Cout == CFG::COUT && H == CFG::HIN && W == CFG::WIN && K == CFG::KS && pad == CFG::PAD) \
        return launch_conv_tc<CFG>(x_act8, wprep, bias, out, stats, N, n_per_view, out_bf16, st);
    TC_RUN(CfgA1) TC_RUN(CfgA2) TC_RUN(CfgA3) TC_RUN(CfgI1) TC_RUN(CfgA1d) TC_RUN(CfgA2d) TC_RUN(CfgA3d) TC_RUN(CfgI1d) TC_RUN(CfgS1) TC_RUN(CfgS1d) TC_RUN(CfgA0) TC_RUN(CfgI0) TC_RUN(CfgS0) TC_RUN(CfgS2) TC_RUN(CfgS2d)
    TC_RUN(CfgB0) TC_RUN(CfgB1) TC_RUN(CfgB1d) TC_RUN(CfgB2) TC_RUN(CfgB2d) TC_RUN(CfgB3) TC_RUN(CfgB3d)
#undef TC_RUN
    set_error("conv_tc: unsupported geometry Cin=%d Cout=%d H=%d W=%d K=%d pad=%d", Cin, Cout, H, W, K, pad);
    return -4;
}

int b200_conv_tc_pool_supported(int Cin, int Cout, int H, int W, int K, int pad) {
#define TC_HAS(CFG) if (Cin == CFG::CIN && Cout == CFG::COUT && H == CFG::HIN && W == CFG::WIN && K == CFG::KS && pad == CFG::PAD) return CFG::POOL_OK ? 1 : 0;
    TC_HAS(CfgA1) TC_HAS(CfgA2) TC_HAS(CfgA3) TC_HAS(CfgI1) TC_HAS(CfgS1) TC_HAS(CfgA0) TC_HAS(CfgI0) TC_HAS(CfgS0) TC_HAS(CfgS2)
    TC_HAS(CfgB0) TC_HAS(CfgB1)
#undef TC_HAS
    return 0;
}

int b200_conv_tc_pool(const void* x_act8, const void* wprep, const float* bias, const float* gamma, void* z_out, void* pool_out, double* stats,
                      int N, int n_per_view, int Cin, int Cout, int H, int W, int K, int pad, int z_fmt, void* stream) {
    B200_REQUIRE(x_act8 && wprep && bias && gamma && pool_out && stats, -1, "conv_tc_pool: null pointer");
    B200_REQUIRE(N > 0 && n_per_view > 0 && N % n_per_view == 0, -2, "conv_tc_pool: N=%d must be a multiple of n_per_view=%d", N, n_per_view);
    B200_REQUIRE(((uintptr_t)x_act8 & 15) == 0 && ((uintptr_t)wprep & 15) == 0 && ((uintptr_t)z_out & 15) == 0 && ((uintptr_t)pool_out & 15) == 0, -3,
                 "conv_tc_pool: pointers must be 16-byte aligned");
    B200_REQUIRE(z_out == nullptr || z_fmt == 1 || z_fmt == 2, -2, "conv_tc_pool: z must be bf16 (1) or fp16 (2) act8");
    cudaStream_t st = as_stream(stream);
#define TC_RUN(CFG) if (Cin == CFG::CIN && Cout == CFG::COUT && H == CFG::HIN && W == CFG::WIN && K == CFG::KS && pad == CFG::PAD) \
        return launch_conv_tc<CFG>(x_act8, wprep, bias, z_out, stats, N, n_per_view, z_fmt, st, pool_out, gamma);
    TC_RUN(CfgA1) TC_RUN(CfgA2) TC_RUN(CfgA3) TC_RUN(CfgI1) TC_RUN(CfgS1) TC_RUN(CfgA0) TC_RUN(CfgI0) TC_RUN(CfgS0)
    TC_RUN(CfgB0) TC_RUN(CfgB1)
#undef TC_RUN
    set_error("conv_tc_pool: unsupported geometry Cin=%d Cout=%d H=%d W=%d K=%d pad=%d", Cin, Cout, H, W, K, pad);
    return -4;
}

int b200_conv_tc_dgrad_bnstat_supported(int Cin, int Cout, int H, int W, int K, int pad) {
#define TC_HAS(CFG) if (Cin == CFG::CIN && Cout == CFG::COUT && H == CFG::HIN && W == CFG::WIN && K == CFG::KS && pad == CFG::PAD) return CFG::BSTAT_OK ? 1 : 0;
    TC_HAS(CfgA1d) TC_HAS(CfgA2d) TC_HAS(CfgA3d) TC_HAS(CfgI1d) TC_HAS(CfgS1d) TC_HAS(CfgS2d)
#undef TC_HAS
    return 0;
}

int b200_conv_tc_dgrad_bnstat(const void* dz_act8, const void* wprep_flip, void* dx_act8, const void* p_act8, const float* gamma, const float* beta,
                              double* sums, int N, int n_per_view, int Cin, int Cout, int H, int W, int K, int pad, void* stream) {
    B200_REQUIRE(dz_act8 && wprep_flip && dx_act8 && p_act8 && gamma && beta && sums, -1, "conv_tc_dgrad_bnstat: null pointer");
    B200_REQUIRE(N > 0 && n_per_view > 0 && N % n_per_view == 0, -2, "conv_tc_dgrad_bnstat: N=%d must be a multiple of n_per_view=%d", N, n_per_view);
    B200_REQUIRE((((uintptr_t)dz_act8 | (uintptr_t)wprep_flip | (uintptr_t)dx_act8) & 15) == 0 && ((uintptr_t)p_act8 & 31) == 0, -3,
                 "conv_tc_dgrad_bnstat: pointers must be 16-byte aligned (p: 32-byte)");
    cudaStream_t st = as_stream(stream);
#define TC_RUN(CFG) if (Cin == CFG::CIN && Cout == CFG::COUT && H == CFG::HIN && W == CFG::WIN && K == CFG::KS && pad == CFG::PAD) \
        return launch_conv_tc<CFG>(dz_act8, wprep_flip, nullptr, dx_act8, sums, N, n_per_view, 1, st, const_cast<void*>(p_act8), gamma, beta);
    TC_RUN(CfgA1d) TC_RUN(CfgA2d) TC_RUN(CfgA3d) TC_RUN(CfgI1d) TC_RUN(CfgS1d) TC_RUN(CfgS2d)
#undef TC_RUN
    set_error("conv_tc_dgrad_bnstat: unsupported geometry Cin=%d Cout=%d H=%d W=%d K=%d pad=%d", Cin, Cout, H, W, K, pad);
    return -4;
}

}
```

multimodal_ssl_avmnist_b200/engine.py:

```python
import contextlib
import math

import numpy as np
import os

import torch

from . import augment as A
from . import dp
from . import ops

F32 = torch.float32


def _conv(n, co, ci, k):
    return [(f"{n}.weight", (co, ci, k, k)), (f"{n}.bias", (co,))]


def _vec2(n, c):
    return [(f"{n}.weight", (c,)), (f"{n}.bias", (c,))]


def _lin(n, o, i):
    return [(f"{n}.weight", (o, i)), (f"{n}.bias", (o,))]


def central_encoder_params(E, O):
    used, unused = [], []
    p = "image_encoder.0"
    used += _conv(f"{p}.conv1", 32, 1, 5) + _vec2(f"{p}.bn1", 32) + _conv(f"{p}.conv2", 64, 32, 5) + _vec2(f"{p}.bn2", 64)
    unused += _lin(f"{p}.fc1", 1024, 1600) + _lin(f"{p}.fc2", 10, 1024)
    used += _lin("image_encoder.1", E, 1600)
    p = "audio_encoder.0"
    used += _conv(f"{p}.conv1", 8, 1, 5) + _vec2(f"{p}.bn1", 8) + _conv(f"{p}.conv2", 16, 8, 5) + _vec2(f"{p}.bn2", 16)
    used += _conv(f"{p}.conv3", 32, 16, 5) + _vec2(f"{p}.bn3", 32) + _conv(f"{p}.conv4", 64, 32, 5) + _vec2(f"{p}.bn4", 64)
    unused += _lin(f"{p}.fc1", 1024, 3136) + _lin(f"{p}.fc2", 10, 1024)
    used += _lin("audio_encoder.1", E, 3136)
    used += _lin("fusion.0", E, 2 * E) + _lin("fusion.3", O, E)
    return used, unused


def central_reference_order(E, O):
    names = []
    p = "image_encoder.0"
    for l in ("conv1", "bn1", "conv2", "bn2", "fc1", "fc2"):
        names += [f"{p}.{l}.weight", f"{p}.{l}.bias"]
    names += ["image_encoder.1.weight", "image_encoder.1.bias"]
    p = "audio_encoder.0"
    for l in ("conv1", "bn1", "conv2", "bn2", "conv3", "bn3", "conv4", "bn4", "fc1", "fc2"):
        names += [f"{p}.{l}.weight", f"{p}.{l}.bias"]
    names += ["audio_encoder.1.weight", "audio_encoder.1.bias", "fusion.0.weight", "fusion.0.bias", "fusion.3.weight", "fusion.3.bias"]
    return names


def image_simple_params(O):
    used = _conv("encoder.0", 32, 1, 3) + _vec2("encoder.1", 32) + _conv("encoder.4", 64, 32, 3) + _vec2("encoder.5", 64)
    used += _conv("encoder.8", 128, 64, 3) + _vec2("encoder.9", 128) + _lin("encoder.14", 512, 128) + _lin("projection.0", O, 512)
    return used, []


def spectrogram_simple_params(O):
    used = []
    for i, (ci, co) in zip((0, 4, 8, 12), ((1, 32), (32, 64), (64, 128), (128, 256))):
        used += _conv(f"encoder.{i}", co, ci, 3) + _vec2(f"encoder.{i + 1}", co)
    used += _lin("encoder.18", O, 256)
    return used, []


def simple_multi_params(E, O, mix=None):
    used = []
    for i, (ci, co) in zip((0, 4, 8), ((1, 32), (32, 64), (64, 128))):
        used += _conv(f"image_encoder.{i}", co, ci, 3) + _vec2(f"image_encoder.{i + 1}", co)
    used += _lin("image_encoder.14", E, 128)
    for i, (ci, co) in zip((0, 4, 8, 12), ((1, 32), (32, 64), (64, 128), (128, 256))):
        used += _conv(f"audio_encoder.{i}", co, ci, 3) + _vec2(f"audio_encoder.{i + 1}", co)
    used += _lin("audio_encoder.18", E, 256)
    used += _lin("fusion.0", E, 2 * E) + _lin("fusion.3", O, E)
    if mix == "gated":
        used += [("gate_image", ()), ("gate_audio", ())]
    elif mix == "cross":
        for a in ("image_to_audio_attention", "audio_to_image_attention"):
            used += _lin(f"{a}.q_proj", E, E) + _lin(f"{a}.kv_proj", 2 * E, E)
    return used, []


def head_params(in_dim, out_dim, hidden=512):
    return _lin("mlp.0", hidden, in_dim) + _vec2("mlp.1", hidden) + _lin("mlp.4", out_dim, hidden)


CENTRAL_IMAGE_LAYERS = [("image_encoder.0.conv1", "image_encoder.0.bn1", 1, 32, 28, 5, 2),
                        ("image_encoder.0.conv2", "image_encoder.0.bn2", 32, 64, 14, 5, 0)]
CENTRAL_AUDIO_LAYERS = [("audio_encoder.0.conv1", "audio_encoder.0.bn1", 1, 8, 112, 5, 2),
                        ("audio_encoder.0.conv2", "audio_encoder.0.bn2", 8, 16, 56, 5, 2),
                        ("audio_encoder.0.conv3", "audio_encoder.0.bn3", 16, 32, 28, 5, 2),
                        ("audio_encoder.0.conv4", "audio_encoder.0.bn4", 32, 64, 14, 5, 2)]
SIMPLE_IMAGE_LAYERS = [("encoder.0", "encoder.1", 1, 32, 28, 3, 1), ("encoder.4", "encoder.5", 32, 64, 14, 3, 1),
                       ("encoder.8", "encoder.9", 64, 128, 7, 3, 1)]
MULTI_SIMPLE_IMAGE_LAYERS = [("image_encoder.0", "image_encoder.1", 1, 32, 28, 3, 1), ("image_encoder.4", "image_encoder.5", 32, 64, 14, 3, 1),
                             ("image_encoder.8", "image_encoder.9", 64, 128, 7, 3, 1)]
MULTI_SIMPLE_AUDIO_LAYERS = [("audio_encoder.0", "audio_encoder.1", 1, 32, 112, 3, 1), ("audio_encoder.4", "audio_encoder.5", 32, 64, 56, 3, 1),
                             ("audio_encoder.8", "audio_encoder.9", 64, 128, 28, 3, 1), ("audio_encoder.12", "audio_encoder.13", 128, 256, 14, 3, 1)]
SPECTROGRAM_LAYERS = [("encoder.0", "encoder.1", 1, 32, 112, 3, 1), ("encoder.4", "encoder.5", 32, 64, 56, 3, 1),
                      ("encoder.8", "encoder.9", 64, 128, 28, 3, 1), ("encoder.12", "encoder.13", 128, 256, 14, 3, 1)]
MULTI_KINDS = {"multi_central": None, "multi_simple": None, "multi_simple_gated": "gated", "multi_cross_attention": "cross"}
UNI_KINDS = {"image_simple": ("img", 128, [("enc.encoder.14", "pool", "e14", 512), ("enc.projection.0", "e14", "feat", None)]),
             "spectrogram_simple": ("aud", 256, [("enc.encoder.18", "pool", "feat", None)])}


class Arena:

    def __init__(self, spec, device, pad_to=4):
        self.spec = list(spec)
        self.offsets = {}
        off = 0
        for name, shape in self.spec:
            n = int(np.prod(shape))
            self.offsets[name] = (off, n, tuple(shape))
            off += (n + pad_to - 1) // pad_to * pad_to
        self.size = off
        self.flat = torch.zeros(max(off, 4), dtype=F32, device=device)

    def view(self, name, flat=None):
        off, n, shape = self.offsets[name]
        return (self.flat if flat is None else flat)[off:off + n].view(shape)

    def views(self, flat=None):
        return {name: self.view(name, flat) for name, _ in self.spec}

    def range_of(self, names):
        lo = min(self.offsets[n][0] for n in names)
        hi = max(self.offsets[n][0] + (self.offsets[n][1] + 3) // 4 * 4 for n in names)
        return lo, hi


class _BN:

    def __init__(self, C, device):
        self.C = C
        self.running_mean = torch.zeros(C, device=device)
        self.running_var = torch.ones(C, device=device)
        self.num_batches_tracked = torch.zeros(1, dtype=torch.int64, device=device)


def _rows(x, n):
    return None if x is None else x[:n]


def _main_chain(fn):
    import functools

    @functools.wraps(fn)
    def wrapped(self, *args, **kwargs):
        with self._on_main():
            return fn(self, *args, **kwargs)
    return wrapped


class DinoStepEngine:

    def __init__(self, kind="multi_central", mode="default", encoder_output_dim=256, output_dim=256, projection_dim=128,
                 n_global_views=2, n_local_views=4, momentum=0.996, center_momentum=0.9, student_temperature=0.1,
                 teacher_temperature=0.04, learning_rate=1e-4, weight_decay=1e-6, dropout=0.3, fusion_dropout=0.3, alpha=1.0,
                 cosine_loss_alpha=0.0, augment_values=None, seed=0, device=None, process_group=None, data_parallel=None,
                 precision="bf16", fused_pool=True, fused_bnstat=False, stream_priorities=False):
        if not torch.cuda.is_available():
            raise ops._lib.B200Error("DinoStepEngine needs a CUDA device: the hot path has no CPU fallback")
        ops._lib.load()
        self.device = torch.device(device if device is not None else f"cuda:{torch.cuda.current_device()}")
        assert kind in MULTI_KINDS or kind in UNI_KINDS
        self.multi = kind in MULTI_KINDS
        self.mix = MULTI_KINDS.get(kind)
        assert mode == "default" or self.multi
        assert precision in ("bf16", "fp32")
        self.precision = precision
        self.lin_tc = precision == "bf16"
        self.kind, self.mode = kind, mode
        self.E, self.O, self.P = encoder_output_dim, output_dim, projection_dim
        self.Vg, self.Vl = n_global_views, n_local_views
        self.V = self.Vg + self.Vl
        self.momentum, self.center_momentum = momentum, center_momentum
        self.tau_s, self.tau_t = student_temperature, teacher_temperature
        self.lr, self.weight_decay = learning_rate, weight_decay
        self.dropout, self.fusion_dropout, self.alpha = dropout, fusion_dropout, alpha
        self.cosine_loss_alpha = cosine_loss_alpha
        self.seed = seed
        self.pg = process_group
        self.world = dp.world_size(process_group) if (data_parallel is None or data_parallel) else 1
        self.step_count = 0
        self.rng_step = 0
        self._loss_slots = [torch.zeros(1).pin_memory() for _ in range(2)]
        self._loss_flip, self._loss_pending = 0, None
        self._ctr = None
        self._bc = None
        self._graph = None

        if kind == "multi_central":
            used, unused = central_encoder_params(self.E, self.O)
            self.img_layers, self.aud_layers = CENTRAL_IMAGE_LAYERS, CENTRAL_AUDIO_LAYERS
            self.top = {"img": (False, 1600, "enc.image_encoder.1"), "aud": (False, 3136, "enc.audio_encoder.1")}
        elif self.multi:
            used, unused = simple_multi_params(self.E, self.O, self.mix)
            self.img_layers, self.aud_layers = MULTI_SIMPLE_IMAGE_LAYERS, MULTI_SIMPLE_AUDIO_LAYERS
            self.top = {"img": (True, 128, "enc.image_encoder.14"), "aud": (True, 256, "enc.audio_encoder.18")}
        elif kind == "image_simple":
            used, unused = image_simple_params(self.O)
            self.img_layers, self.aud_layers = SIMPLE_IMAGE_LAYERS, []
            self.top = {}
        else:
            used, unused = spectrogram_simple_params(self.O)
            self.img_layers, self.aud_layers = [], SPECTROGRAM_LAYERS
            self.top = {}
        self.uni = UNI_KINDS.get(kind)
        head = [("head." + n, s) for n, s in head_params(self.O, self.P)]
        enc_used = [("enc." + n, s) for n, s in used]
        enc_unused = [("enc." + n, s) for n, s in unused]
        aux = []
        if mode != "default":
            out = 10 if mode == "semi_supervised" else self.P
            for m in ("aux_image", "aux_audio"):
                aux += [(f"{m}.{n}", s) for n, s in head_params(self.E, out)]
        self.student = Arena(enc_used + head + enc_unused + aux, self.device)
        self.teacher = Arena(enc_used + head + enc_unused, self.device)
        self.n_ema = self.teacher.size
        self.n_trainable_prefix = self.student.range_of([n for n, _ in enc_used + head])[1]
        self.aux_range = self.student.range_of([n for n, _ in aux]) if aux else None
        self.grad_plan = dp.GradientPlan([(0, self.n_trainable_prefix)] + ([self.aux_range] if self.aux_range else []))
        self._bucket_split = self.student.offsets[self.top["aud"][2] + ".weight"][0] if self.multi else 0
        self._grad_scale = 1.0
        self.grad = torch.zeros_like(self.student.flat)
        self.exp_avg = torch.zeros_like(self.student.flat)
        self.exp_avg_sq = torch.zeros_like(self.student.flat)
        self.S = self.student.views()
        self.T = self.teacher.views()
        self.G = self.student.views(self.grad)
        self.center = torch.zeros(1, self.P, device=self.device)
        self.bn_s, self.bn_t = {}, {}
        for conv, bn, ci, co, hw, k, pad in self.img_layers + self.aud_layers:
            self.bn_s["enc." + bn], self.bn_t["enc." + bn] = _BN(co, self.device), _BN(co, self.device)
        self.bn_s["head.mlp.1"], self.bn_t["head.mlp.1"] = _BN(512, self.device), _BN(512, self.device)
        for m in ("aux_image", "aux_audio"):
            if aux:
                self.bn_s[f"{m}.mlp.1"] = _BN(512, self.device)
        self.tc = {}
        for mod, layers in (("img", self.img_layers), ("aud", self.aud_layers)):
            self.tc[mod] = [precision == "bf16" and ops.conv_tc_supported(ci, co, hw, hw, k, pad) and
                            (ci == 1 or ops.conv_tc_supported(co, ci, hw + 2 * pad - k + 1, hw + 2 * pad - k + 1, k, k - 1 - pad))
                            for (conv, bn, ci, co, hw, k, pad) in layers]
        for mod in self.tc:
            if self.tc[mod] and self.tc[mod][0] and not (len(self.tc[mod]) > 1 and self.tc[mod][1]):
                self.tc[mod][0] = False
        self.fused_pool = bool(fused_pool) and kind in ("multi_central", "image_simple")
        self.pool = {}
        for role in ("s", "t"):
            self.pool[role] = {mod: [self.fused_pool and bool(self.tc[mod][li]) and ops.conv_tc_pool_supported(ci, co, hw, hw, k, pad)
                                     and (role == "t" or (ci == 1 and hw >= 112))
                                     for li, (conv, bn, ci, co, hw, k, pad) in enumerate(layers)]
                               for mod, layers in (("img", self.img_layers), ("aud", self.aud_layers))}
        self.fused_bnstat = bool(fused_bnstat)
        self.bnstat = {mod: [self.fused_bnstat and li > 0 and bool(self.tc[mod][li]) and bool(self.tc[mod][li - 1]) and
                             ops.conv_tc_dgrad_bnstat_supported(co, ci, hw + 2 * pad - k + 1, hw + 2 * pad - k + 1, k, k - 1 - pad)
                             for li, (conv, bn, ci, co, hw, k, pad) in enumerate(layers)]
                       for mod, layers in (("img", self.img_layers), ("aud", self.aud_layers))}
        self._tcw = {}
        self._prep_desc = {}
        for mod, layers in (("img", self.img_layers), ("aud", self.aud_layers)):
            for li, (conv, bn, ci, co, hw, k, pad) in enumerate(layers):
                if self.tc[mod][li]:
                    for role in ("s", "t"):
                        self._tcw[(role, mod, li)] = torch.empty(ops.conv_tc_weight_bytes(ci, co, k), dtype=torch.uint8, device=self.device)
                    if ci > 1:
                        self._tcw[("flip", mod, li)] = torch.empty(ops.conv_tc_weight_bytes(co, ci, k), dtype=torch.uint8, device=self.device)
        self.overlap_teacher = True
        lo, hi = 0, -1
        try:
            hi = int(os.environ.get("B200_TOP_PRIORITY", "-3"))
        except ValueError:
            pass
        self.stream_priorities = bool(stream_priorities)

        def mk(level):
            return torch.cuda.Stream(device=self.device, priority=(min(lo, hi + level) if self.stream_priorities else 0))

        self._main_stream = mk(0) if self.stream_priorities else None
        self._side_stream = mk(1)
        self._lin_wg_stream = mk(3)
        self._lin_wg_pending = False
        self._side_stream2 = mk(1)
        self._wgrad_streams = {m: mk(2) for m in ("img", "aud")}
        self._aug_stream = mk(3)
        self.comm = dp.AbiComm.get(process_group) if self.world > 1 else None
        self._comm_stream = torch.cuda.Stream(device=self.device) if self.world > 1 else None
        self.overlap_grad_exchange = False
        self._center_ready = None
        self._comm_pending = False
        self._prefetch, self._step_done, self._step_done_prev = None, None, None
        self._eval_wrole = "s"
        self._ws = {}
        self._init_parameters()
        self.set_augmentation(augment_values)

    @contextlib.contextmanager
    def _on_main(self):
        hp = self._main_stream
        cur = torch.cuda.current_stream()
        if hp is None or cur == hp:
            yield
            return
        hp.wait_stream(cur)
        with torch.cuda.stream(hp):
            yield
        cur.wait_stream(hp)

    def _init_parameters(self):
        g = torch.Generator(device="cpu").manual_seed(self.seed)
        bn_bases = {"enc." + bn for _, bn, *_ in self.img_layers + self.aud_layers} | {"head.mlp.1", "aux_image.mlp.1", "aux_audio.mlp.1"}
        bounds = {}
        for name, shape in self.student.spec:
            v = self.student.view(name)
            base = name.rsplit(".", 1)[0]
            if base in bn_bases:
                v.fill_(1.0 if name.endswith(".weight") else 0.0)
            elif len(shape) == 0:
                v.fill_(0.5)
            elif len(shape) > 1:
                bounds[base] = 1.0 / math.sqrt(int(np.prod(shape[1:])))
                v.copy_(((torch.rand(shape, generator=g) * 2 - 1) * bounds[base]).to(self.device))
            else:
                v.copy_(((torch.rand(shape, generator=g) * 2 - 1) * bounds[base]).to(self.device))
        self.sync_teacher()

    def sync_teacher(self):
        self.teacher.flat.copy_(self.student.flat[:self.n_ema])
        for k in self.bn_t:
            self.bn_t[k].running_mean.copy_(self.bn_s[k].running_mean)
            self.bn_t[k].running_var.copy_(self.bn_s[k].running_var)
            self.bn_t[k].num_batches_tracked.copy_(self.bn_s[k].num_batches_tracked)

    def load_named(self, student=None, teacher=None, student_head=None, teacher_head=None, aux_image=None, aux_audio=None):
        for prefix, arena_views, src in (("enc.", self.S, student), ("enc.", self.T, teacher), ("head.", self.S, student_head),
                                         ("head.", self.T, teacher_head), ("aux_image.", self.S, aux_image), ("aux_audio.", self.S, aux_audio)):
            if src is None:
                continue
            for k, v in src.items():
                if prefix + k in arena_views:
                    arena_views[prefix + k].copy_(v.to(self.device))

    def set_augmentation(self, augment_values):
        ig, il = A.image_chains()
        ag, al = A.default_audio_chains() if augment_values is None else A.audio_chains_from_values(augment_values)
        self.chains = (ig, il, ag, al)
        spec = np.stack([A.pack_spec(c) for c in self.chains])
        self.aug_spec = torch.from_numpy(spec).to(self.device)

    def _workspace(self, B):
        if B in self._ws:
            return self._ws[B]
        dev, V, Vg = self.device, self.V, self.Vg
        if self.world > 1:
            lohi = torch.tensor([B, -B], dtype=torch.int64, device=dev)
            torch.distributed.all_reduce(lohi, op=torch.distributed.ReduceOp.MAX, group=self.pg)
            if int(lohi[0]) != B or int(-lohi[1]) != B:
                raise ops._lib.B200Error(f"data parallel: per-rank batch sizes differ ({int(-lohi[1])}..{int(lohi[0])}); use equal shards "
                                         "(drop_last) -- the gradient average and the centre EMA weight every rank equally")
        extra = 1 if self.mode != "default" else 0
        Ns, Nt = (V + extra) * B, Vg * B

        def e(*shape, dtype=F32):
            return torch.empty(*shape, dtype=dtype, device=dev)

        w = {"B": B, "Ns": Ns, "Nt": Nt}
        zarena = torch.zeros(1 << 17, dtype=torch.float64, device=dev)
        zoff = [0]

        def zalloc(*shape):
            n = int(math.prod(shape))
            o = zoff[0]
            zoff[0] = o + (n + 1) // 2 * 2
            if zoff[0] > zarena.numel():
                raise ops._lib.B200Error("zero arena too small")
            return zarena[o:o + n].view(*shape)

        w["zarena"] = zarena
        if self.img_layers:
            w["img_ops"] = torch.zeros(B, V, A.MAX_OPS, A.OP_WORDS, dtype=torch.int32, device=dev)
        w["aud_ops"] = torch.zeros(B, V, A.MAX_OPS, A.OP_WORDS, dtype=torch.int32, device=dev)
        w["group_bits"] = torch.zeros(B, V, A.GROUP_WORDS, dtype=torch.int32, device=dev)
        for nm in ("img_ops", "aud_ops", "group_bits"):
            if nm in w:
                w[nm + "_b"] = torch.zeros_like(w[nm])
        if self.img_layers:
            w["x_img"] = e(Ns, 1, 28, 28)
        if self.aud_layers:
            w["x_aud"] = e(Ns, 1, 112, 112)
        scr = {m: dict(wg=0, z=0, p=0, z8=0) for m in ("img", "aud")}
        BF = torch.bfloat16
        for role, N in (("s", Ns), ("t", Nt)):
            for mod, layers in (("img", self.img_layers), ("aud", self.aud_layers)):
                for li, (conv, bn, ci, co, hw, k, pad) in enumerate(layers):
                    ho = hw + 2 * pad - k + 1
                    nv = N // B
                    tc = self.tc[mod][li]
                    next_tc = li + 1 < len(layers) and self.tc[mod][li + 1]
                    if tc and ci == 1 and role == "s":
                        wq = ops.quad8_width(hw, pad)
                        w[f"{mod}.xs8"] = e(N, hw, wq, 8, dtype=BF)
                        w[f"{mod}.xs8_b"] = e(N, hw, wq, 8, dtype=BF)
                    pooled = tc and self.pool[role][mod][li]
                    if pooled:
                        w[f"{role}.{mod}.e{li}"] = e(N, co // 8, ho // 2, ho // 2, 8, dtype=torch.float16)
                    if tc and (role == "s" or not pooled):
                        w[f"{role}.{mod}.z{li}"] = e(N, co // 8, ho, ho, 8, dtype=torch.float16)
                    elif not tc:
                        w[f"{role}.{mod}.z{li}"] = e(N, co, ho, ho)
                    if next_tc:
                        w[f"{role}.{mod}.p8{li}"] = e(N, co // 8, ho // 2, ho // 2, 8, dtype=BF)
# ... 247 lines not shown
                xa = w["aud.xs8"][:V * B].view(V, B, 112, ops.quad8_width(112, pa), 8)
                ops.aug_apply_audio(audios.reshape(B, 112, 112), aud_ops, group_bits, None, noise=noise, seed=seed, out8=xa, pad=pa,
                                    step_dev=step_dev)
            return xi, xa
        xi = xa = None
        if self.img_layers:
            xi = w["x_img"][:V * B].view(V, B, 28, 28)
            ops.aug_apply_image(images.reshape(B, 28, 28), img_ops, xi)
        if self.aud_layers and audios is not None:
            xa = w["x_aud"][:V * B].view(V, B, 112, 112)
            ops.aug_apply_audio(audios.reshape(B, 112, 112), aud_ops, group_bits, xa, noise=noise, seed=seed, step_dev=step_dev)
        return xi, xa

    def _prep_tc_weights(self, role, P):
        desc = self._prep_desc.get(role)
        if desc is None:
            rows = []
            for mod, layers in (("img", self.img_layers), ("aud", self.aud_layers)):
                for li, (conv, bn, ci, co, hw, k, pad) in enumerate(layers):
                    if self.tc[mod][li]:
                        wt = P["enc." + conv + ".weight"]
                        rows.append([wt.data_ptr(), self._tcw[(role, mod, li)].data_ptr(), ci, co, k, 0])
                        if role == "s" and ci > 1:
                            rows.append([wt.data_ptr(), self._tcw[("flip", mod, li)].data_ptr(), co, ci, k, 1])
            desc = torch.tensor(rows, dtype=torch.int64, device=self.device) if rows else False
            self._prep_desc[role] = desc
        if desc is not False:
            ops.conv_tc_prep_weights_multi(desc)

    def _conv_stack(self, w, role, mod, layers, x, N, B, P, bns, train=True):
        nv = N // B
        cur = x
        for li, (conv, bn, ci, co, hw, k, pad) in enumerate(layers):
            z, stats = w.get(f"{role}.{mod}.z{li}"), w[f"{role}.{mod}.stats{li}"]
            tc = self.tc[mod][li]
            next_tc = li + 1 < len(layers) and self.tc[mod][li + 1]
            pooled = tc and self.pool["s" if role == "s" else "t"][mod][li]
            if "zarena" not in w:
                stats.zero_()
            wrole = role if role in ("s", "t") else self._eval_wrole
            if tc:
                xin = cur
                if ci == 1:
                    xs8 = w[f"{mod}.xs8"]
                    if role == "s" and not w.get("packed", False):
                        ops.pack_quad8(cur.view(N, hw, hw), xs8, pad)
                    xin = xs8[:N]
                if pooled:
                    ops.conv_tc_pool(xin, self._tcw[(wrole, mod, li)], P["enc." + conv + ".bias"], P["enc." + bn + ".weight"],
                                     z if role == "s" else None, w[f"{role}.{mod}.e{li}"], stats, B, co, k, pad)
                else:
                    ops.conv_tc(xin, self._tcw[(wrole, mod, li)], P["enc." + conv + ".bias"], z, stats, B, co, k, pad)
            else:
                ops.conv_fwd(cur.view(N, ci, hw, hw), P["enc." + conv + ".weight"], P["enc." + conv + ".bias"], z, stats, B, pad)
            b = bns["enc." + bn]
            ho = hw + 2 * pad - k + 1
            sc, sh = w[f"{role}.{mod}.scale{li}"], w[f"{role}.{mod}.shift{li}"]
            ops.bn_finalize(stats, P["enc." + bn + ".weight"], P["enc." + bn + ".bias"], b.running_mean, b.running_var,
                            b.num_batches_tracked, sc, sh, w[f"{role}.{mod}.mean{li}"], w[f"{role}.{mod}.invstd{li}"], nv, B * ho * ho, train=train)
            if tc:
                cur = w[f"{role}.{mod}.p8{li}"] if next_tc else w[f"{role}.{mod}.p{li}"]
                if pooled:
                    ops.bn_relu_apply8(w[f"{role}.{mod}.e{li}"], sc, sh, cur, B)
                else:
                    ops.bn_relu_pool8_fwd(z, sc, sh, cur, B)
            else:
                cur = w[f"{role}.{mod}.p{li}"]
                ops.bn_relu_pool_fwd(z, sc, sh, cur, B)
                if next_tc:
                    ops.pack_act8(cur, w[f"{role}.{mod}.p8{li}"])
                    cur = w[f"{role}.{mod}.p8{li}"]
        return cur

    def _head_fwd(self, w, role, prefix, P, bn, x, out, hh, g, mask, drop_p, tag=""):
        M = x.shape[0]
        ops.linear_fwd(x, P[prefix + "mlp.0.weight"], P[prefix + "mlp.0.bias"], hh, tc=self.lin_tc)
        st = w[f"{role}.{tag}hstats"]
        if "zarena" not in w:
            st.zero_()
        ops.colstats(hh, st)
        ops.bn_finalize(st, P[prefix + "mlp.1.weight"], P[prefix + "mlp.1.bias"], bn.running_mean, bn.running_var, bn.num_batches_tracked,
                        w[f"{role}.{tag}hscale"], w[f"{role}.{tag}hshift"], w[f"{role}.{tag}hmean"], w[f"{role}.{tag}hinvstd"], 1, M)
        ops.bn1d_gelu_drop_fwd(hh, w[f"{role}.{tag}hscale"], w[f"{role}.{tag}hshift"], mask, drop_p, g)
        ops.linear_fwd(g, P[prefix + "mlp.4.weight"], P[prefix + "mlp.4.bias"], out, tc=self.lin_tc)

    def _lin_wgrad(self, dy, x, gw, gb):
        st = self._lin_wg_stream if self.overlap_teacher else None
        if st is None:
            ops.linear_bwd_weight(dy, x, gw, gb, tc=self.lin_tc)
            return
        st.wait_stream(torch.cuda.current_stream())
        with torch.cuda.stream(st):
            ops.linear_bwd_weight(dy, x, gw, gb, tc=self.lin_tc)
        self._lin_wg_pending = True

    def _head_bwd(self, w, role, prefix, x, d_out, hh, g, d_g, d_hh, d_x, mask, drop_p, tag=""):
        S, G = self.S, self.G
        self._lin_wgrad(d_out, g, G[prefix + "mlp.4.weight"], G[prefix + "mlp.4.bias"])
        ops.linear_bwd_data(d_out, S[prefix + "mlp.4.weight"], d_g, tc=self.lin_tc)
        sums = w[f"{role}.{tag}hsums"]
        if "zarena" not in w:
            sums.zero_()
        sc, sh, mu, inv = (w[f"{role}.{tag}h{n}"] for n in ("scale", "shift", "mean", "invstd"))
        ops.bn1d_gelu_drop_bwd_reduce(hh, d_g, sc, sh, mu, inv, mask, drop_p, sums)
        ops.bn1d_gelu_drop_bwd_apply(hh, d_g, sc, sh, mu, inv, mask, drop_p, sums, d_hh)
        ops.bn_param_grads(sums, G[prefix + "mlp.1.weight"], G[prefix + "mlp.1.bias"], 1)
        self._lin_wgrad(d_hh, x, G[prefix + "mlp.0.weight"], G[prefix + "mlp.0.bias"])
        ops.linear_bwd_data(d_hh, S[prefix + "mlp.0.weight"], d_x, tc=self.lin_tc)

    def _encode(self, w, role, P, bns, x_img, x_aud, N, B, n_fusion, fmask, train=True):
        if self.multi:
            E = self.E
            catr = w[f"{role}.catr"]

            def top(mod, p_last, cols):
                pool, nflat, lin = self.top[mod]
                if pool:
                    ops.avgpool_fwd(p_last, w[f"{role}.{mod}.gap"])
                    x = w[f"{role}.{mod}.gap"]
                else:
                    x = p_last.view(N, nflat)
                ops.linear_fwd(x, P[lin + ".weight"], P[lin + ".bias"], catr[:, cols], tc=self.lin_tc)

            main = torch.cuda.current_stream()
            side = self._side_stream2 if (self.overlap_teacher and role == "s") else None
            if side is not None:
                side.wait_stream(main)
            with (torch.cuda.stream(side) if side is not None else contextlib.nullcontext()):
                pi = self._conv_stack(w, role, "img", self.img_layers, x_img, N, B, P, bns, train=train)
                top("img", pi, slice(0, E))
            pa = self._conv_stack(w, role, "aud", self.aud_layers, x_aud, N, B, P, bns, train=train)
            if side is not None:
                main.wait_stream(side)
            top("aud", pa, slice(E, 2 * E))
            self._mix_fwd(w, role, P, n_fusion, B)
            cat = w[f"{role}.cat"]
            h1, feat = w[f"{role}.h1"], w[f"{role}.feat"]
            if fmask is None:
                ops.linear_fwd(cat[:n_fusion], P["enc.fusion.0.weight"], P["enc.fusion.0.bias"], h1, act=1, tc=self.lin_tc)
            else:
                ops.linear_fwd(cat[:n_fusion], P["enc.fusion.0.weight"], P["enc.fusion.0.bias"], h1, act=2, mask=fmask, drop_p=self.fusion_dropout, tc=self.lin_tc)
            ops.linear_fwd(h1, P["enc.fusion.3.weight"], P["enc.fusion.3.bias"], feat, tc=self.lin_tc)
            return feat
        mod, _, chain = self.uni
        p_last = self._conv_stack(w, role, mod, self._layers(mod), x_img if mod == "img" else x_aud, N, B, P, bns, train=train)
        ops.avgpool_fwd(p_last, w[f"{role}.pool"])
        for lin, src, dst, _ in chain:
            ops.linear_fwd(w[f"{role}.{src}"], P[lin + ".weight"], P[lin + ".bias"], w[f"{role}.{dst}"], tc=self.lin_tc)
        return w[f"{role}.feat"]

    def _layers(self, mod):
        return self.img_layers if mod == "img" else self.aud_layers

    def _conv_stack_bwd(self, w, mod, layers, x, d_top, N, B):
        S, G = self.S, self.G
        d_p = d_top
        BF = torch.bfloat16
        if any(self.tc[mod]) and "zarena" not in w:
            w[f"{mod}.dbsum"].zero_()
        main = torch.cuda.current_stream()
        wside = self._wgrad_streams[mod] if self.overlap_teacher else None
        busy = {}
        for li in range(len(layers) - 1, -1, -1):
            conv, bn, ci, co, hw, k, pad = layers[li]
            ho = hw + 2 * pad - k + 1
            tc = self.tc[mod][li]
            z = w[f"s.{mod}.z{li}"]
            sums = w[f"s.{mod}.sums{li}"]
            if "zarena" not in w:
                sums.zero_()
            sc, sh, mu, inv = (w[f"s.{mod}.{n}{li}"] for n in ("scale", "shift", "mean", "invstd"))
            if tc:
                if d_p.dtype != BF:
                    d_p = d_p.view(N, co, ho // 2, ho // 2)
                par = li & 1
                if par in busy:
                    main.wait_event(busy.pop(par))
                fused = ci == 1
                if not fused:
                    dz = w[f"{mod}.dz8" if par == 0 else f"{mod}.dz8b"][:z.numel()].view_as(z)
                p_out = w[f"s.{mod}.p8{li}"] if f"s.{mod}.p8{li}" in w else w[f"s.{mod}.p{li}"]
                if not (li + 1 < len(layers) and self.bnstat[mod][li + 1]):
                    ops.bn_pool8_bwd_reduce_p(p_out, d_p, S["enc." + bn + ".weight"], S["enc." + bn + ".bias"], sums, B)
                if not fused:
                    ops.bn_relu_pool8_bwd_apply(z, d_p, sc, sh, mu, inv, sums, dz, B, dbsum=w[f"{mod}.dbsum"][li])
            else:
                dz = w[f"{mod}.dz"][:z.numel()].view_as(z)
                ops.bn_relu_pool_bwd_reduce(z, d_p, sc, sh, mu, inv, sums, B)
                ops.bn_relu_pool_bwd_apply(z, d_p, sc, sh, mu, inv, sums, dz, B)

            def param_grads(li=li, tc=tc, fused=tc and ci == 1, conv=conv, bn=bn, sums=sums):
                if tc and not fused:
                    ops.bias_grad_finalize(w[f"{mod}.dbsum"][li], G["enc." + conv + ".bias"])
                ops.bn_param_grads(sums, G["enc." + bn + ".weight"], G["enc." + bn + ".bias"], N // B)

            if not (tc and wside is not None):
                param_grads()
            if tc:
                xin8 = w[f"{mod}.xs8"] if ci == 1 else w[f"s.{mod}.p8{li - 1}"]
                wk = w[f"{mod}.wg_work" if (li & 1) == 0 else f"{mod}.wg_work_b"]

                def wgrad():
                    if wside is not None:
                        param_grads()
                    if fused:
                        ops.conv_tc_wgrad_l0_fused(xin8, z, d_p, sc, sh, mu, inv, sums, G["enc." + conv + ".weight"], w[f"{mod}.dbsum"][li], wk,
                                                   B, pad)
                        ops.bias_grad_finalize(w[f"{mod}.dbsum"][li], G["enc." + conv + ".bias"])
                    else:
                        ops.conv_tc_wgrad(xin8, dz, G["enc." + conv + ".weight"], wk, pad)

                if wside is not None:
                    wside.wait_stream(main)
                    with torch.cuda.stream(wside):
                        wgrad()
                        ev = torch.cuda.Event()
                        ev.record(wside)
                    busy[li & 1] = ev
                else:
                    wgrad()
            else:
                xin = x if li == 0 else w[f"s.{mod}.p{li - 1}"]
                ops.conv_bwd_weight(xin.view(N, ci, hw, hw), dz, G["enc." + conv + ".weight"], G["enc." + conv + ".bias"], w[f"{mod}.wg_work"], pad)
            if li > 0:
                nxt = w[f"{mod}.dp_a"] if d_p.data_ptr() != w[f"{mod}.dp_a"].data_ptr() else w[f"{mod}.dp_b"]
                if tc:
                    if self.tc[mod][li - 1]:
                        d_in = nxt.view(BF)[:N * ci * hw * hw].view(N, ci // 8, hw, hw, 8)
                    else:
                        d_in = nxt[:N * ci * hw * hw].view(N, ci, hw, hw)
                    if self.bnstat[mod][li]:
                        lbn = layers[li - 1][1]
                        ops.conv_tc_dgrad_bnstat(dz, self._tcw[("flip", mod, li)], d_in, w[f"s.{mod}.p8{li - 1}"], S["enc." + lbn + ".weight"],
                                                 S["enc." + lbn + ".bias"], w[f"s.{mod}.sums{li - 1}"], B, k, k - 1 - pad)
                    else:
                        ops.conv_tc(dz, self._tcw[("flip", mod, li)], None, d_in, None, N, ci, k, k - 1 - pad)
                else:
                    d_in = nxt[:N * ci * hw * hw].view(N, ci, hw, hw)
                    ops.conv_bwd_data(dz, S["enc." + conv + ".weight"], d_in, pad)
                d_p = d_in
        if wside is not None:
            main.wait_stream(wside)

    def _eval_workspace(self, B):
        key = ("eval", B)
        if key in self._ws:
            return self._ws[key]
        dev, BF = self.device, torch.bfloat16
        w = {"B": B}

        def e(*shape, dtype=F32):
            return torch.empty(*shape, dtype=dtype, device=dev)

        if self.img_layers:
            w["x_img"] = e(B, 1, 28, 28)
        if self.aud_layers:
            w["x_aud"] = e(B, 1, 112, 112)
        for mod, layers in (("img", self.img_layers), ("aud", self.aud_layers)):
            for li, (conv, bn, ci, co, hw, k, pad) in enumerate(layers):
                ho = hw + 2 * pad - k + 1
                tc = self.tc[mod][li]
                next_tc = li + 1 < len(layers) and self.tc[mod][li + 1]
                if tc and ci == 1:
                    w[f"{mod}.xs8"] = e(B, hw, ops.quad8_width(hw, pad), 8, dtype=BF)
                if tc and self.pool["t"][mod][li]:
                    w[f"e.{mod}.e{li}"] = e(B, co // 8, ho // 2, ho // 2, 8, dtype=torch.float16)
                else:
                    w[f"e.{mod}.z{li}"] = e(B, co // 8, ho, ho, 8, dtype=torch.float16) if tc else e(B, co, ho, ho)
                if next_tc:
                    w[f"e.{mod}.p8{li}"] = e(B, co // 8, ho // 2, ho // 2, 8, dtype=BF)
                if not next_tc or not tc:
                    w[f"e.{mod}.p{li}"] = e(B, co, ho // 2, ho // 2)
                w[f"e.{mod}.stats{li}"] = torch.zeros(1, co, 2, dtype=torch.float64, device=dev)
                for nm in ("scale", "shift", "mean", "invstd"):
                    w[f"e.{mod}.{nm}{li}"] = e(1, co)
        E, O = self.E, self.O
        if self.multi:
            self._mix_workspace(w, "e", B, B, B, e)
            w["e.h1"], w["e.feat"] = e(B, E), e(B, O)
            w["e.fmask"] = torch.ones(B, E, dtype=torch.uint8, device=dev)
            for mod in ("img", "aud"):
                if self.top[mod][0]:
                    w[f"e.{mod}.gap"] = e(B, self.top[mod][1])
        else:
            self._uni_workspace(w, "e", B, e)
        self._ws[key] = w
        return w

    def begin_probe(self, teacher=False):
        src = self.bn_t if teacher else self.bn_s
        bns = {}
        for k, v in src.items():
            c = _BN(v.C, self.device)
            c.running_mean.copy_(v.running_mean)
            c.running_var.copy_(v.running_var)
            c.num_batches_tracked.copy_(v.num_batches_tracked)
            bns[k] = c
        return {"bns": bns, "step": 0, "teacher": teacher}

    @_main_chain
    @torch.no_grad()
    def encode_features(self, images, audios=None, train=False, teacher=False, probe=None):
        B = self._batch_size(images, audios)
        w = self._eval_workspace(B)
        P = self.T if teacher else self.S
        bns = self.bn_t if teacher else self.bn_s
        if probe is not None:
            bns = probe["bns"]
        elif train:
            bns = {k: _BN(v.C, self.device) for k, v in bns.items()}
        xi = xa = None
        if self.img_layers:
            xi = w["x_img"]
            xi.copy_((images.float() / 255.0 if images.dtype == torch.uint8 else images).reshape(B, 1, 28, 28))
        if self.aud_layers:
            xa = w["x_aud"]
            xa.copy_((audios.float() / 255.0 if audios.dtype == torch.uint8 else audios).reshape(B, 1, 112, 112))
        w["packed"] = False
        if self._tcw:
            self._prep_tc_weights("t" if teacher else "s", P)
        for mod, layers, x in (("img", self.img_layers, xi), ("aud", self.aud_layers, xa)):
            if layers and self.tc[mod][0]:
                ops.pack_quad8(x.view(B, layers[0][4], layers[0][4]), w[f"{mod}.xs8"], layers[0][6])
        w["packed"] = True
        fmask = None
        if train and self.multi and self.fusion_dropout > 0:
            fmask = w["e.fmask"]
            if probe is not None:
                probe["step"] += 1
            ops.dropout_mask(fmask, self.fusion_dropout, self.seed + 17, (self.rng_step + (probe["step"] if probe is not None else 0)) * 4 + 3)
        self._eval_wrole = "t" if teacher else "s"
        return self._encode(w, "e", P, bns, xi, xa, B, B, B, fmask, train=train)

    @_main_chain
    def forward_pass(self, x_img, x_aud, masks=None, raw=None):
        V, Vg, E = self.V, self.Vg, self.E
        x_in = x_img if self.img_layers else x_aud
        B = x_in.shape[1]
        w = self._workspace(B)
        Ns, Nt, Nv = w["Ns"], w["Nt"], V * B
        S, T = self.S, self.T
        multi = self.multi
        xi = w.get("x_img")
        xa = w.get("x_aud")
        self._join_center()
        w["zarena"].zero_()
        packed = x_in.dtype == torch.bfloat16
        w["packed"] = packed
        if packed:
            if ((self.img_layers and x_img.data_ptr() != w["img.xs8"].data_ptr()) or
                    (self.aud_layers and x_aud.data_ptr() != w["aud.xs8"].data_ptr())):
                raise ops._lib.B200Error("bf16 inputs must be the workspace quad8 images returned by augment(direct=True)")
            if self.mode != "default":
                ops.pack_quad8(raw[0].reshape(B, 28, 28), w["img.xs8"][Nv:], self.img_layers[0][6])
                ops.pack_quad8(raw[1].reshape(B, 112, 112), w["aud.xs8"][Nv:], self.aud_layers[0][6])
        else:
            if self.img_layers and x_img.data_ptr() != xi.data_ptr():
                xi[:Nv].copy_(x_img.reshape(Nv, 1, 28, 28))
            if self.aud_layers and x_aud.data_ptr() != xa.data_ptr():
                xa[:Nv].copy_(x_aud.reshape(Nv, 1, 112, 112))
            if self.mode != "default":
                xi[Nv:].copy_(raw[0].reshape(B, 1, 28, 28))
                xa[Nv:].copy_(raw[1].reshape(B, 1, 112, 112))
        if masks is not None:
            if multi:
                w["s.fmask"].copy_(masks["student_fusion"].reshape(Nv, E))
                w["t.fmask"].copy_(masks["teacher_fusion"].reshape(Nt, E))
            w["s.hmask"].copy_(masks["student_head"].reshape(Nv, 512))
        else:
            step, step_dev = self._step_args()
            base = step * 4
            if multi:
                ops.dropout_mask(w["s.fmask"], self.fusion_dropout, self.seed + 1, base, step_dev=step_dev)
                ops.dropout_mask(w["t.fmask"], self.fusion_dropout, self.seed + 1, base + 1, step_dev=step_dev)
            if self.dropout > 0:
                ops.dropout_mask(w["s.hmask"], self.dropout, self.seed + 1, base + 2, step_dev=step_dev)
        if self._tcw:
            self._prep_tc_weights("s", S)
            self._prep_tc_weights("t", T)
        if not packed:
            for mod, layers, x in (("img", self.img_layers, xi), ("aud", self.aud_layers, xa)):
                if layers and self.tc[mod][0]:
                    hw, pad = layers[0][4], layers[0][6]
                    ops.pack_quad8(x.view(Ns, hw, hw), w[f"{mod}.xs8"], pad)
            w["packed"] = True
        main = torch.cuda.current_stream()
        side = self._side_stream if self.overlap_teacher else None
        if side is not None:
            side.wait_stream(main)
            with torch.cuda.stream(side):
# ... 369 lines not shown
```

multimodal_ssl_avmnist_b200/ops.py:

```python
import torch

from . import _lib


def _lib_():
    return _lib.load()


def _ptr(t, dtype=None):
    if t is None:
        return None
    if not t.is_cuda:
        raise _lib.B200Error("B200 ops need CUDA tensors (there is no CPU fallback)")
    if not t.is_contiguous():
        raise _lib.B200Error("B200 ops need contiguous tensors")
    if dtype is not None and t.dtype != dtype:
        raise _lib.B200Error(f"expected {dtype}, got {t.dtype}")
    return t.data_ptr()


_RAW_STREAM = getattr(torch._C, "_cuda_getCurrentRawStream", None)
_GET_DEVICE = getattr(torch._C, "_cuda_getDevice", None)


# ... 117 lines not shown
                                       _ptr(loss_out, F32), _ptr(work, F32), _stream()), "ce_fwd_bwd")


def infonce_work_floats(B, D, tc=False):
    return (_lib_().b200_infonce_tc_work_floats if tc else _lib_().b200_infonce_work_floats)(B, D)


def infonce_fwd_bwd(a, b, grad_a, grad_b, loss_out, work, temperature=0.07, grad_scale=1.0, tc=False):
    B, D = a.shape
    fn = _lib_().b200_infonce_fwd_bwd_tc if tc else _lib_().b200_infonce_fwd_bwd
    _lib.check(fn(_ptr(a, F32), _ptr(b, F32), B, D, temperature, grad_scale, _ptr(grad_a, F32), _ptr(grad_b, F32), _ptr(loss_out, F32),
                  _ptr(work, F32), _stream()), "infonce_fwd_bwd")


def ntxent_work_floats(N, D):
    return int(_lib_().b200_ntxent_work_floats(N, D))


def ntxent_fwd_bwd(reps, grad, loss_out, work, temperature=0.07, grad_scale=1.0):
    N, D = reps.shape
    _lib.check(_lib_().b200_ntxent_fwd_bwd(_ptr(reps, F32), N, D, temperature, grad_scale, _ptr(grad, F32), _ptr(loss_out, F32),
                                           _ptr(work, F32), _stream()), "ntxent_fwd_bwd")


def cosine_consistency_fwd_bwd(emb, grad_emb, loss_out, grad_scale=1.0, work=None):
    V, B, D = emb.shape
    work = _loss_work(emb.device, B) if work is None else work
    _lib.check(_lib_().b200_cosine_consistency_fwd_bwd(_ptr(emb, F32), V, B, D, grad_scale, _ptr(grad_emb, F32), _ptr(loss_out, F32),
                                                       _ptr(work, F32), _stream()), "cosine_consistency_fwd_bwd")


def _aug_outs(out, out8, pad):
    ref = out if out is not None else out8
    if ref is None:
        raise _lib.B200Error("augmentation needs an fp32 and / or a quad8 output")
    return ref.shape[0], ref.shape[1], (_ptr(out, F32) if out is not None else None), (_ptr(out8, torch.bfloat16) if out8 is not None else None)


def aug_apply_image(src, ops, out, out8=None, pad=0, elastic_grid=None, seed=0):
    V, B, po, p8 = _aug_outs(out, out8, pad)
    _lib.check(_lib_().b200_aug_apply_image_ex(_ptr(src), 1 if src.dtype == U8 else 0, _ptr(ops, I32), _ptr(elastic_grid, F32), seed, po, p8, pad,
                                               B, V, _stream()), "aug_apply_image")


def aug_apply_audio(src, ops, group_bits, out, noise=None, seed=0, out8=None, pad=0, step_dev=None):
    V, B, po, p8 = _aug_outs(out, out8, pad)
    _lib.check(_lib_().b200_aug_apply_audio_dev(_ptr(src), 1 if src.dtype == U8 else 0, _ptr(ops, I32), _ptr(group_bits, I32),
                                                _ptr(noise, F32), seed, _ptr(step_dev, I64), po, p8, pad, B, V, _stream()), "aug_apply_audio")


def aug_sample(spec, B, Vg, Vl, seed, step, img_ops, aud_ops, group_bits, step_dev=None):
    _lib.check(_lib_().b200_aug_sample_dev(_ptr(spec, I32), B, Vg, Vl, seed, step, _ptr(step_dev, I64), _ptr(img_ops, I32),
                                           _ptr(aud_ops, I32), _ptr(group_bits, I32), _stream()), "aug_sample")


def conv_supported(Cin, Cout, H, W, K, pad):
    return bool(_lib_().b200_conv_supported(Cin, Cout, H, W, K, pad))


def conv_fwd(x, w, bias, z, stats, n_per_view, pad):
    N, Cin, H, W = x.shape
    Cout, _, K, _ = w.shape
    _lib.check(_lib_().b200_conv_fwd(_ptr(x, F32), _ptr(w, F32), _ptr(bias, F32), _ptr(z, F32), _ptr(stats, F64), N, n_per_view, Cin,
                                     Cout, H, W, K, pad, _stream()), "conv_fwd")


def conv_bwd_data(dz, w, dx, pad):
    N, Cin, H, W = dx.shape
    Cout, _, K, _ = w.shape
    _lib.check(_lib_().b200_conv_bwd_data(_ptr(dz, F32), _ptr(w, F32), _ptr(dx, F32), N, Cin, Cout, H, W, K, pad, _stream()), "conv_bwd_data")


def conv_bwd_weight_work_floats(N, Cin, Cout, H, W, K, pad):
    n = _lib_().b200_conv_bwd_weight_work_floats(N, Cin, Cout, H, W, K, pad)
    if n < 0:
        raise _lib.B200Error(f"conv_bwd_weight: shape {(Cin, Cout, H, W, K, pad)} not compiled")
    return n


def conv_bwd_weight(x, dz, dw, db, work, pad):
    N, Cin, H, W = x.shape
    Cout, _, K, _ = dw.shape
    _lib.check(_lib_().b200_conv_bwd_weight(_ptr(x, F32), _ptr(dz, F32), _ptr(dw, F32), _ptr(db, F32), _ptr(work, F32), N, Cin, Cout, H, W,
                                            K, pad, _stream()), "conv_bwd_weight")


BF16 = torch.bfloat16


def conv_tc_supported(Cin, Cout, H, W, K, pad):
    return bool(_lib_().b200_conv_tc_supported(Cin, Cout, H, W, K, pad))


def conv_tc_weight_bytes(Cin, Cout, K):
    return int(_lib_().b200_conv_tc_weight_bytes(Cin, Cout, K))


def conv_tc_prep_weights(w, wprep, flip=False):
    Co, Ci, K, _ = w.shape
    cin, cout = (Co, Ci) if flip else (Ci, Co)
    _lib.check(_lib_().b200_conv_tc_prep_weights(_ptr(w, F32), _ptr(wprep), cin, cout, K, 1 if flip else 0, _stream()), "conv_tc_prep_weights")


def pack_act8(x, out):
    N, Cc, H, W = x.shape
    _lib.check(_lib_().b200_pack_act8(_ptr(x, F32), _ptr(out, BF16), N, Cc, H, W, _stream()), "pack_act8")


def conv_tc(x8, wprep, bias, out, stats, n_per_view, Cout, K, pad):
    if x8.dim() == 4:
        N, H, WQ, _ = x8.shape
        W = out.shape[-1 if out.dim() == 4 else -2] - 2 * pad + K - 1
        if WQ != quad8_width(W, pad):
            raise _lib.B200Error(f"conv_tc: quad8 input of width {WQ} does not match W={W}, pad={pad}")
        P = 0.125
    else:
        N, P, H, W, _ = x8.shape
    fmt = 1 if out.dtype == BF16 else 2 if out.dtype == torch.float16 else 0
    _lib.check(_lib_().b200_conv_tc(_ptr(x8, BF16), _ptr(wprep), _ptr(bias, F32) if bias is not None else None, _ptr(out),
                                    _ptr(stats, F64) if stats is not None else None, N, n_per_view, int(P * 8), Cout, H, W, K, pad,
                                    fmt, _stream()), "conv_tc")


def conv_tc_pool_supported(Cin, Cout, H, W, K, pad):
    return bool(_lib_().b200_conv_tc_pool_supported(Cin, Cout, H, W, K, pad))


def conv_tc_pool(x8, wprep, bias, gamma, z_out, pool_out, stats, n_per_view, Cout, K, pad):
    Wo = pool_out.shape[-2] * 2
    if x8.dim() == 4:
        N, H, WQ, _ = x8.shape
        W = Wo - 2 * pad + K - 1
        if WQ != quad8_width(W, pad):
            raise _lib.B200Error(f"conv_tc_pool: quad8 input of width {WQ} does not match W={W}, pad={pad}")
        Cin = 1
    else:
        N, P, H, W, _ = x8.shape
        Cin = P * 8
    fmt = 0 if z_out is None else (1 if z_out.dtype == BF16 else 2)
    _lib.check(_lib_().b200_conv_tc_pool(_ptr(x8, BF16), _ptr(wprep), _ptr(bias, F32), _ptr(gamma, F32), _ptr(z_out) if z_out is not None else None,
                                         _ptr(pool_out, torch.float16), _ptr(stats, F64), N, n_per_view, Cin, Cout, H, W, K, pad, fmt, _stream()),
               "conv_tc_pool")


def conv_tc_dgrad_bnstat_supported(Cin, Cout, H, W, K, pad):
    return bool(_lib_().b200_conv_tc_dgrad_bnstat_supported(Cin, Cout, H, W, K, pad))


def conv_tc_dgrad_bnstat(dz8, wprep_flip, dx8, p8, gamma, beta, sums, n_per_view, K, pad):
    N, P, H, W, _ = dz8.shape
    Cout = dx8.shape[1] * 8
    _lib.check(_lib_().b200_conv_tc_dgrad_bnstat(_ptr(dz8, BF16), _ptr(wprep_flip), _ptr(dx8, BF16), _ptr(p8, BF16), _ptr(gamma, F32), _ptr(beta, F32),
                                                 _ptr(sums, F64), N, n_per_view, P * 8, Cout, H, W, K, pad, _stream()), "conv_tc_dgrad_bnstat")


def bn_relu_apply8(e8, scale, shift, out, n_per_view):
    N, P, HP, WP, _ = e8.shape
    _lib.check(_lib_().b200_bn_relu_apply8(_ptr(e8, torch.float16), _ptr(scale, F32), _ptr(shift, F32), _ptr(out), N, n_per_view, P * 8, HP, WP,
                                           _fmt(out), _stream()), "bn_relu_apply8")


def conv_tc_prep_weights_multi(desc):
    _lib.check(_lib_().b200_conv_tc_prep_weights_multi(_ptr(desc, torch.int64), desc.shape[0], _stream()), "conv_tc_prep_weights_multi")


def conv_tc_wgrad_variant(tap=-1):
    return int(_lib_().b200_conv_tc_wgrad_variant(tap))


def conv_tc_wgrad_work_floats(N, Cin, Cout, H, W, K, pad):
    n = int(_lib_().b200_conv_tc_wgrad_work_floats(N, Cin, Cout, H, W, K, pad))
    if n < 0:
        raise _lib.B200Error(f"conv_tc_wgrad: unsupported geometry {(Cin, Cout, H, W, K, pad)}")
    return n


def conv_tc_wgrad(x8, dz8, dw, work, pad):
    N, H, W = x8.shape[0], x8.shape[-3], x8.shape[-2]
    Cout, Cin, K, _ = dw.shape
    if Cin == 1:
        W -= pad
    _lib.check(_lib_().b200_conv_tc_wgrad(_ptr(x8, BF16), _ptr(dz8, BF16), _ptr(dw, F32), _ptr(work, F32), N, Cin, Cout, H, W, K, pad,
                                          _stream()), "conv_tc_wgrad")


def conv_tc_wgrad_l0_fused_work_floats(N, n_per_view, Cout, H, W, K, pad):
    n = int(_lib_().b200_conv_tc_wgrad_l0_fused_work_floats(N, n_per_view, Cout, H, W, K, pad))
    if n < 0:
        raise _lib.B200Error(f"conv_tc_wgrad_l0_fused: unsupported geometry {(Cout, H, W, K, pad)}")
    return n


def conv_tc_wgrad_l0_fused(xs8, z8, dp8, scale, shift, mean, invstd, sums, dw, dbsum, work, n_per_view, pad):
    N, P, H, W, _ = z8.shape
    Cout, _, K, _ = dw.shape
    _lib.check(_lib_().b200_conv_tc_wgrad_l0_fused(_ptr(xs8, BF16), _ptr(z8, torch.float16), _ptr(dp8, BF16), _ptr(scale, F32), _ptr(shift, F32),
                                                   _ptr(mean, F32), _ptr(invstd, F32), _ptr(sums, F64), _ptr(dw, F32),
                                                   _ptr(dbsum, F64) if dbsum is not None else None, _ptr(work, F32), N, n_per_view, Cout, H, W,
                                                   K, pad, _stream()), "conv_tc_wgrad_l0_fused")


def quad8_width(W, pad):
    return (W + 2 * pad + 3) // 4


def pack_quad8(x, out, pad):
    N, H, W = x.shape[0], x.shape[-2], x.shape[-1]
    assert tuple(out.shape) == (N, H, quad8_width(W, pad), 8)
    _lib.check(_lib_().b200_pack_quad8(_ptr(x, F32), _ptr(out, BF16), N, H, W, pad, _stream()), "pack_quad8")


def pack_shift8(x, out, pad):
    N, H, W = x.shape[0], x.shape[-2], x.shape[-1]
    assert tuple(out.shape) == (N, H, W + pad, 8)
    _lib.check(_lib_().b200_pack_shift8(_ptr(x, F32), _ptr(out, BF16), N, H, W, pad, _stream()), "pack_shift8")


def bias_grad_finalize(dbsum, db):
    _lib.check(_lib_().b200_bias_grad_finalize(_ptr(dbsum, F64), _ptr(db, F32), db.numel(), _stream()), "bias_grad_finalize")


def unpack_act8(x8, out):
    N, P, H, W, _ = x8.shape
    _lib.check(_lib_().b200_unpack_act8(_ptr(x8, BF16), _ptr(out, F32), N, P * 8, H, W, _stream()), "unpack_act8")


def _fmt(t):
    return 1 if t.dtype == BF16 else 0


def _zf16(z8):
    if z8.dtype not in (BF16, torch.float16):
        raise _lib.B200Error(f"act8 z must be bf16 or fp16, got {z8.dtype}")
    return 1 if z8.dtype == torch.float16 else 0


def bn_relu_pool8_fwd(z8, scale, shift, out, n_per_view):
    N, P, H, W, _ = z8.shape
    _lib.check(_lib_().b200_bn_relu_pool8_fwd(_ptr(z8), _ptr(scale, F32), _ptr(shift, F32), _ptr(out), N, n_per_view, P * 8, H, W,
                                              _zf16(z8), _fmt(out), _stream()), "bn_relu_pool8_fwd")


def bn_relu_pool8_bwd_reduce(z8, dp, scale, shift, mean, invstd, sums, n_per_view):
    N, P, H, W, _ = z8.shape
    _lib.check(_lib_().b200_bn_relu_pool8_bwd_reduce(_ptr(z8), _ptr(dp), _ptr(scale, F32), _ptr(shift, F32), _ptr(mean, F32),
                                                     _ptr(invstd, F32), _ptr(sums, F64), N, n_per_view, P * 8, H, W, _zf16(z8), _fmt(dp), _stream()),
               "bn_relu_pool8_bwd_reduce")


def bn_pool8_bwd_reduce_p(p, dp, gamma, beta, sums, n_per_view):
    if p.dim() == 5:
        N, P, HP, WP, _ = p.shape
        Cc = P * 8
    else:
        N, Cc, HP, WP = p.shape
    _lib.check(_lib_().b200_bn_pool8_bwd_reduce_p(_ptr(p), _ptr(dp), _ptr(gamma, F32), _ptr(beta, F32), _ptr(sums, F64), N, n_per_view, Cc,
                                                  HP, WP, _fmt(p), _fmt(dp), _stream()), "bn_pool8_bwd_reduce_p")


def bn_relu_pool8_bwd_apply(z8, dp, scale, shift, mean, invstd, sums, dz8, n_per_view, dbsum=None):
    N, P, H, W, _ = z8.shape
    _lib.check(_lib_().b200_bn_relu_pool8_bwd_apply(_ptr(z8), _ptr(dp), _ptr(scale, F32), _ptr(shift, F32), _ptr(mean, F32),
                                                    _ptr(invstd, F32), _ptr(sums, F64), _ptr(dz8, BF16),
                                                    _ptr(dbsum, F64) if dbsum is not None else None, N, n_per_view, P * 8, H, W, _zf16(z8),
                                                    _fmt(dp), _stream()), "bn_relu_pool8_bwd_apply")


def bn_finalize(stats, gamma, beta, running_mean, running_var, nbt, scale, shift, mean, invstd, n_views, count, train=True,
                momentum=0.1, eps=1e-5):
    Cc = gamma.numel()
    _lib.check(_lib_().b200_bn_finalize(_ptr(stats, F64), _ptr(gamma, F32), _ptr(beta, F32), _ptr(running_mean, F32), _ptr(running_var, F32),
                                        _ptr(nbt, I64), _ptr(scale, F32), _ptr(shift, F32), _ptr(mean, F32), _ptr(invstd, F32), n_views,
                                        Cc, count, momentum, eps, 1 if train else 0, _stream()), "bn_finalize")


def bn_relu_pool_fwd(z, scale, shift, out, n_per_view):
    N, Cc, H, W = z.shape
    _lib.check(_lib_().b200_bn_relu_pool_fwd(_ptr(z, F32), _ptr(scale, F32), _ptr(shift, F32), _ptr(out, F32), N, n_per_view, Cc, H, W,
                                             _stream()), "bn_relu_pool_fwd")


def bn_relu_pool_bwd_reduce(z, dout, scale, shift, mean, invstd, sums, n_per_view):
    N, Cc, H, W = z.shape
    _lib.check(_lib_().b200_bn_relu_pool_bwd_reduce(_ptr(z, F32), _ptr(dout, F32), _ptr(scale, F32), _ptr(shift, F32), _ptr(mean, F32),
                                                    _ptr(invstd, F32), _ptr(sums, F64), N, n_per_view, Cc, H, W, _stream()),
               "bn_relu_pool_bwd_reduce")


def bn_relu_pool_bwd_apply(z, dout, scale, shift, mean, invstd, sums, dz, n_per_view):
    N, Cc, H, W = z.shape
    _lib.check(_lib_().b200_bn_relu_pool_bwd_apply(_ptr(z, F32), _ptr(dout, F32), _ptr(scale, F32), _ptr(shift, F32), _ptr(mean, F32),
                                                   _ptr(invstd, F32), _ptr(sums, F64), _ptr(dz, F32), N, n_per_view, Cc, H, W, _stream()),
               "bn_relu_pool_bwd_apply")


def bn_param_grads(sums, dgamma, dbeta, n_views, accumulate=False):
    _lib.check(_lib_().b200_bn_param_grads(_ptr(sums, F64), _ptr(dgamma, F32), _ptr(dbeta, F32), n_views, dgamma.numel(),
                                           1 if accumulate else 0, _stream()), "bn_param_grads")


def avgpool_fwd(x, out):
    N, Cc = x.shape[0], x.shape[1]
    _lib.check(_lib_().b200_avgpool_fwd(_ptr(x, F32), _ptr(out, F32), N, Cc, x[0, 0].numel(), _stream()), "avgpool_fwd")


def avgpool_bwd(dout, dx):
    N, Cc = dx.shape[0], dx.shape[1]
    _lib.check(_lib_().b200_avgpool_bwd(_ptr(dout, F32), _ptr(dx, F32), N, Cc, dx[0, 0].numel(), _stream()), "avgpool_bwd")


def _rows(t):
    if not t.is_cuda or t.dtype != F32 or t.dim() != 2 or t.stride(1) != 1:
        raise _lib.B200Error("linear ops need 2-D fp32 CUDA tensors with unit column stride")
    return t.data_ptr(), t.stride(0)


def linear_fwd(x, w, bias, y, act=0, mask=None, drop_p=0.0, tc=False):
    M, K = x.shape
    N = w.shape[0]
    xp, ldx = _rows(x)
    yp, ldy = _rows(y)
    fn = _lib_().b200_linear_fwd_tc if tc else _lib_().b200_linear_fwd
    _lib.check(fn(xp, ldx, _ptr(w, F32), _ptr(bias, F32), yp, ldy, M, N, K, act, _ptr(mask, U8), drop_p, _stream()), "linear_fwd")


_LINEAR_WORK = {}


def _linear_work(device, need):
    key = (device, _stream())
    work = _LINEAR_WORK.get(key)
    if work is None or work.numel() < need:
        work = _LINEAR_WORK[key] = torch.empty(max(need, 4), dtype=F32, device=device)
    return work


def linear_bwd_data(dy, w, dx, tc=False):
    M, N = dy.shape
    K = w.shape[1]
    dyp, lddy = _rows(dy)
    dxp, lddx = _rows(dx)
    if tc:
        work = _linear_work(dy.device, _lib_().b200_linear_bwd_data_tc_work_floats(M, N, K))
        _lib.check(_lib_().b200_linear_bwd_data_tc(dyp, lddy, _ptr(w, F32), dxp, lddx, _ptr(work, F32), M, N, K, _stream()), "linear_bwd_data")
    else:
        _lib.check(_lib_().b200_linear_bwd_data(dyp, lddy, _ptr(w, F32), dxp, lddx, M, N, K, _stream()), "linear_bwd_data")


def linear_bwd_weight(dy, x, dw, db, accumulate=False, work=None, tc=False):
    M, N = dy.shape
    K = x.shape[1]
    dyp, lddy = _rows(dy)
    xp, ldx = _rows(x)
    need = (_lib_().b200_linear_bwd_weight_tc_work_floats if tc else _lib_().b200_linear_bwd_weight_work_floats)(M, N, K)
    if work is None and need > 0:
        work = _linear_work(dy.device, need)
    fn = _lib_().b200_linear_bwd_weight_tc if tc else _lib_().b200_linear_bwd_weight
    _lib.check(fn(dyp, lddy, xp, ldx, _ptr(dw, F32), _ptr(db, F32), _ptr(work, F32), M, N, K, 1 if accumulate else 0, _stream()),
               "linear_bwd_weight")


def gate_apply(x, gate, y):
    M, N = x.shape
    xp, ldx = _rows(x)
    yp, ldy = _rows(y)
    _lib.check(_lib_().b200_gate_apply(xp, ldx, yp, ldy, _ptr(gate, F32), M, N, _stream()), "gate_apply")


def gate_grad_work_floats():
    return int(_lib_().b200_gate_grad_work_floats())


def gate_grad(dy, x, gate, dgate, work, accumulate=False):
    M, N = x.shape
    dyp, lddy = _rows(dy)
    xp, ldx = _rows(x)
    _lib.check(_lib_().b200_gate_grad(dyp, lddy, xp, ldx, _ptr(gate, F32), _ptr(dgate, F32), _ptr(work, F32), M, N, 1 if accumulate else 0,
                                      _stream()), "gate_grad")


def softmax_rows(s, scale):
    M, N = s.shape
    sp, ld = _rows(s)
    _lib.check(_lib_().b200_softmax_rows(sp, ld, M, N, scale, _stream()), "softmax_rows")


def softmax_rows_bwd(dp, p, scale):
    M, N = p.shape
    dpp, lddp = _rows(dp)
    pp, ldp = _rows(p)
    _lib.check(_lib_().b200_softmax_rows_bwd(dpp, lddp, pp, ldp, M, N, scale, _stream()), "softmax_rows_bwd")


def add2d(dst, src):
    M, N = dst.shape
    dp, ldd = _rows(dst)
    sp, lds = _rows(src)
    _lib.check(_lib_().b200_add2d(dp, ldd, sp, lds, M, N, _stream()), "add2d")


def act_bwd(dy, y, drop_p=0.0):
    _lib.check(_lib_().b200_act_bwd(_ptr(dy, F32), _ptr(y, F32), None, drop_p, dy.numel(), _stream()), "act_bwd")


def colstats(h, stats):
    M, Cc = h.shape
    _lib.check(_lib_().b200_colstats(_ptr(h, F32), _ptr(stats, F64), M, Cc, _stream()), "colstats")


def bn1d_gelu_drop_fwd(h, scale, shift, mask, drop_p, g):
    M, Cc = h.shape
    _lib.check(_lib_().b200_bn1d_gelu_drop_fwd(_ptr(h, F32), _ptr(scale, F32), _ptr(shift, F32), _ptr(mask, U8), drop_p, _ptr(g, F32), M, Cc,
                                               _stream()), "bn1d_gelu_drop_fwd")


def bn1d_gelu_drop_bwd_reduce(h, dg, scale, shift, mean, invstd, mask, drop_p, sums):
    M, Cc = h.shape
    _lib.check(_lib_().b200_bn1d_gelu_drop_bwd_reduce(_ptr(h, F32), _ptr(dg, F32), _ptr(scale, F32), _ptr(shift, F32), _ptr(mean, F32),
                                                      _ptr(invstd, F32), _ptr(mask, U8), drop_p, _ptr(sums, F64), M, Cc, _stream()),
               "bn1d_gelu_drop_bwd_reduce")


def bn1d_gelu_drop_bwd_apply(h, dg, scale, shift, mean, invstd, mask, drop_p, sums, dh):
    M, Cc = h.shape
    _lib.check(_lib_().b200_bn1d_gelu_drop_bwd_apply(_ptr(h, F32), _ptr(dg, F32), _ptr(scale, F32), _ptr(shift, F32), _ptr(mean, F32),
                                                     _ptr(invstd, F32), _ptr(mask, U8), drop_p, _ptr(sums, F64), _ptr(dh, F32), M, Cc,
                                                     _stream()), "bn1d_gelu_drop_bwd_apply")


def knn_predict(train_feats, train_labels, test_feats, k=5, n_classes=10, return_neighbours=False, chunk=2048):
    N, D = train_feats.shape
    M = test_feats.shape[0]
    dev = train_feats.device
    bias = torch.empty(N, dtype=F32, device=dev)
    tp, ldt = _rows(train_feats)
    _lib.check(_lib_().b200_knn_neg_half_sqnorm(tp, ldt, N, D, _ptr(bias, F32), _stream()), "knn_neg_half_sqnorm")
    pred = torch.empty(M, dtype=I64, device=dev)
    nbr = torch.empty(M, k, dtype=I32, device=dev) if return_neighbours else None
    scores = torch.empty(min(chunk, M), N, dtype=F32, device=dev)
    labels = train_labels.to(I64).contiguous()
    for lo in range(0, M, chunk):
        hi = min(M, lo + chunk)
        linear_fwd(test_feats[lo:hi], train_feats, bias, scores[:hi - lo])
        _lib.check(_lib_().b200_knn_topk_vote(_ptr(scores, F32), N, _ptr(labels, I64), hi - lo, N, k, n_classes, pred[lo:hi].data_ptr(),
                                              nbr[lo:hi].data_ptr() if nbr is not None else None, _stream()), "knn_topk_vote")
    return (pred, nbr) if return_neighbours else pred


_LAUNCHES = {"gate_grad": 2, "ntxent_fwd_bwd": 5, "conv_tc_wgrad_l0_fused": 3, "conv_tc_wgrad": 2, "conv_bwd_weight": 3, "linear_bwd_weight": 3, "infonce_fwd_bwd": 9}
_NOT_KERNELS = {"conv_tc_wgrad_variant", "gate_grad_work_floats", "knn_predict", "conv_tc_pool_supported", "conv_tc_dgrad_bnstat_supported", "quad8_width", "ntxent_work_floats", "conv_tc_wgrad_l0_fused_work_floats", "conv_tc_wgrad_work_floats", "conv_tc_supported", "conv_tc_weight_bytes", "dino_loss_parts", "infonce_work_floats", "conv_supported", "conv_bwd_weight_work_floats", "launch_count", "start_profile", "stop_profile"}
LAUNCH_COUNT = 0
_PROFILE = None


def launch_count():
    return LAUNCH_COUNT


def start_profile():
    global _PROFILE
    _PROFILE = []
    return _PROFILE


def stop_profile():
    global _PROFILE
    rec, _PROFILE = _PROFILE, None
    return rec


_LAUNCHES_TC = {"linear_bwd_weight": 6, "linear_bwd_data": 2, "infonce_fwd_bwd": 19}


def _wrap(name, fn):
    n_launch = _LAUNCHES.get(name, 1)
    n_launch_tc = _LAUNCHES_TC.get(name, n_launch)

    def wrapped(*args, **kwargs):
        global LAUNCH_COUNT
        LAUNCH_COUNT += n_launch_tc if kwargs.get("tc") else n_launch
        if _PROFILE is None:
            return fn(*args, **kwargs)
        a, b = torch.cuda.Event(enable_timing=True), torch.cuda.Event(enable_timing=True)
        a.record()
        out = fn(*args, **kwargs)
        b.record()
        head = args[:6] if name == "conv_tc_pool" else args[:4]
        meta = tuple(tuple(t.shape) for t in list(head) + list(kwargs.values()) if isinstance(t, torch.Tensor))
        meta = meta + (("i",) + tuple(int(v) for v in args if isinstance(v, int) and not isinstance(v, bool)),)
        _PROFILE.append((name, a, b, meta, _stream()))
        return out

    wrapped.__name__ = name
    wrapped.__doc__ = fn.__doc__
    return wrapped


for _name, _fn in list(globals().items()):
    if callable(_fn) and not _name.startswith("_") and _name not in _NOT_KERNELS and getattr(_fn, "__module__", None) == __name__ \
            and _name not in ("launch_count", "start_profile", "stop_profile", "MultiTensorTable"):
        globals()[_name] = _wrap(_name, _fn)
```

Baseline: 135,100.

## Fuse BatchNorm/ReLU/pool backward apply into tensor-core data-gradient conv

Adds a variant of the tensor-core conv kernel with an extra 128-thread warpgroup. That warpgroup takes each TMA-loaded pre-activation tile from shared memory, applies the BN+ReLU+maxpool backward in place, and writes dz to global memory. It also accumulates the bias-gradient sums before the MMA issuer consumes the tile through a new ready barrier. The goal is to remove the separate bn_relu_pool8_bwd_apply kernel launch and its full read/write of z and dz, since the data-gradient conv now reads z directly. It is enabled by default for multi_central layers with li>0 whose geometry fits. The cost is more threads and shared memory per CTA, plus an extra serial stage inside the conv pipeline.

```diff
diff --git a/include/avmnist_b200.h b/include/avmnist_b200.h
--- a/include/avmnist_b200.h
+++ b/include/avmnist_b200.h
@@ -95,6 +95,10 @@
 int b200_conv_tc_dgrad_bnstat(const void* dz_act8, const void* wprep_flip, void* dx_act8, const void* p_act8, const float* gamma,
                               const float* beta, double* sums, int N, int n_per_view, int Cin, int Cout, int H, int W, int K,
                               int pad, void* stream);
+int b200_conv_tc_dgrad_bnapply_supported(int Cin, int Cout, int H, int W, int K, int pad);
+int b200_conv_tc_dgrad_bnapply(const void* z8, const void* dp, const float* scale, const float* shift, const float* mean, const float* invstd,
+                               const double* sums, const void* wprep_flip, void* dx_act8, void* dz8, double* dbsum, int N, int n_per_view,
+                               int Cin, int Cout, int H, int W, int K, int pad, int dp_fmt, void* stream);
 int b200_bn_relu_apply8(const void* e8, const float* scale, const float* shift, void* out, int N, int n_per_view, int C, int HP,
                         int WP, int out_fmt, void* stream);
 int b200_bn_relu_pool8_fwd(const void* z8, const float* scale, const float* shift, void* out, int N, int n_per_view,
diff --git a/multimodal_ssl_avmnist_b200/contrastive.py b/multimodal_ssl_avmnist_b200/contrastive.py
--- a/multimodal_ssl_avmnist_b200/contrastive.py
+++ b/multimodal_ssl_avmnist_b200/contrastive.py
@@ -70,6 +70,8 @@
         self.pool["t"] = self.pool["s"]
         self.fused_bnstat = False
         self.bnstat = {mod: [False] * len(layers) for mod, layers in (("img", IMG_LAYERS), ("aud", AUD_LAYERS))}
+        self.fused_bwd_apply = False
+        self.bnapply = {mod: [False] * len(layers) for mod, layers in (("img", IMG_LAYERS), ("aud", AUD_LAYERS))}
         self._tcw, self._prep_desc = {}, {}
         for mod, layers in (("img", IMG_LAYERS), ("aud", AUD_LAYERS)):
             for li, (conv, bn, ci, co, hw, k, pad) in enumerate(layers):
diff --git a/multimodal_ssl_avmnist_b200/csrc/conv_tc.cu b/multimodal_ssl_avmnist_b200/csrc/conv_tc.cu
--- a/multimodal_ssl_avmnist_b200/csrc/conv_tc.cu
+++ b/multimodal_ssl_avmnist_b200/csrc/conv_tc.cu
@@ -126,6 +126,33 @@
     static_assert(HO % BANDS == 0, "bands must divide the output height");
     static_assert(SMEM <= 227 * 1024, "shared memory budget");
     static_assert(XPL * PHASE_BYTES < (1 << 18) && PLANE_BYTES % 16 == 0, "descriptor range");
+    static constexpr bool BNA_OK = CIN_ > COUT_ && CIN_ <= 64 && NSPLIT_ == 1 && KCH_ == 1 && HIN_ % 2 == 0 && WIN_ % 2 == 0 && PAD_ % 2 == 0 &&
+                                   HB % 2 == 0 && (BANDS_ == 1 || HO == HIN_) && (XPH == 1 || XPH % 2 == 0);
+    static constexpr int BNA_TPO = 128 / P;
+    static constexpr int BNA_NW = (HIN / 2 < HPB / 2 ? HIN / 2 : HPB / 2) * (WIN / 2);
+    static constexpr int BNA_IT = (BNA_NW + BNA_TPO - 1) / BNA_TPO;
+    static constexpr int BNA_SEG = BNA_TPO < 32 ? BNA_TPO : 32;
+    static constexpr int BNA_OFF = round_up(SMEM_NOPOOL, 16);
+    static constexpr int SMEM_BNA = BNA_OFF + CIN * 16 + (128 / BNA_SEG) * 8 * 4;
+    static_assert(!BNA_OK || (3 * SLOTS + 2 * NBUF <= 24 && (SMEM_BNA + 1024) * CTAS <= 227 * 1024), "BNA barriers / shared memory");
+};
+
+__device__ __forceinline__ int argmax4_first(float y0, float y1, float y2, float y3, float& m) {
+    int k = 0;
+    m = y0;
+    if (y1 > m) { m = y1; k = 1; }
+    if (y2 > m) { m = y2; k = 2; }
+    if (y3 > m) { m = y3; k = 3; }
+    return k;
+}
+
+struct BnaArgs {
+    const void* dp;
+    const float *scale, *shift, *mean, *invstd;
+    const double* sums;
+    uint4* dz;
+    double* dbsum;
+    int n_per_view;
 };
 
 __device__ __forceinline__ void ld_global_nc_256(const uint4* p, uint4& a, uint4& b) {
@@ -152,11 +179,13 @@
     }
 }
 
-template <class C, bool POOL, bool BSTAT = false>
-__global__ void __launch_bounds__(C::THREADS, C::CTAS)
+template <class C, bool POOL, bool BSTAT = false, int BNA = 0>
+__global__ void __launch_bounds__(C::THREADS + (BNA ? 128 : 0), C::CTAS)
 conv_tc_kernel(const __grid_constant__ TMaps tmaps, const uint4* __restrict__ wprep, const float* __restrict__ bias,
                void* __restrict__ out, double* __restrict__ stats, int n_per_view, int out_bf16,
-               uint4* __restrict__ pool_out, const float* __restrict__ gamma, const float* __restrict__ beta2 = nullptr) {
+               uint4* __restrict__ pool_out, const float* __restrict__ gamma, const float* __restrict__ beta2 = nullptr,
+               const BnaArgs bna = BnaArgs()) {
+    static_assert(!BNA || (C::BNA_OK && !POOL && !BSTAT), "BNA: data-gradient instances only");
     extern __shared__ __align__(1024) uint8_t smem[];
     uint8_t* w_s = smem;
     uint8_t* img_s = smem + C::W_BYTES;
@@ -177,6 +206,7 @@
     auto empty_bar = [&](int s) { return bar0 + 8u * (C::SLOTS + s); };
     auto tfull_bar = [&](int b) { return bar0 + 8u * (2 * C::SLOTS + b); };
     auto tempty_bar = [&](int b) { return bar0 + 8u * (2 * C::SLOTS + C::NBUF + b); };
+    auto ready_bar = [&](int s) { return bar0 + 8u * (2 * C::SLOTS + 2 * C::NBUF + s); };
 
     {
         const uint4* src = wprep;
@@ -221,6 +251,8 @@
             mbar_init(tfull_bar(b), 1);
             mbar_init(tempty_bar(b), 4);
         }
+        if constexpr (BNA != 0)
+            for (int s = 0; s < C::SLOTS; ++s) mbar_init(ready_bar(s), 128);
         fence_mbar_init();
     }
     if (warp == 1) tmem_alloc<C::TMEM_COLS>(smem_u32(tmem_slot));
@@ -229,6 +261,7 @@
     tc_fence_after_sync();
     const uint32_t tmem_base = *tmem_slot;
     const uint32_t img_addr = smem_u32(img_s), w_addr = smem_u32(w_s);
+    constexpr int EPI_END = C::ISS + 4;
 
     if (warp == 0) {
         if (lane == 0) {
@@ -256,7 +289,7 @@
 #pragma unroll 1
               for (int c = 0; c < C::KCH; ++c) {
                 const int k = (i - i0) * C::KCH + c, slot = k % C::SLOTS, use = k / C::SLOTS;
-                mbar_wait(full_bar(slot), use & 1);
+                mbar_wait(BNA ? ready_bar(slot) : full_bar(slot), use & 1);
                 tc_fence_after_sync();
                 const uint32_t slot_addr = img_addr + slot * C::SLOT_BYTES;
                 for (int t = warp - 1; t < C::TILES; t += C::ISS) {
@@ -308,7 +341,7 @@
               }
             }
         }
-    } else {
+    } else if (warp <= EPI_END) {
         const int quad = warp & 3, row = quad * 32 + lane;
         float s1[C::COUTL], s2[C::COUTL];
 #pragma unroll
@@ -368,7 +401,7 @@
                             f[j] = __uint_as_float(v[j]);
                         } else {
                             f[j] = __uint_as_float(v[j]) + bias_s[col];
-                            if (col < C::XPH * C::COUTL && valid) {
+                            if (!BNA && col < C::XPH * C::COUTL && valid) {
                                 s1[ch] += f[j];
                                 s2[ch] += f[j] * f[j];
                             }
@@ -506,7 +539,7 @@
                 }
             }
         }
-        if (do_stats) {
+        if (!BNA && do_stats) {
 #pragma unroll
             for (int c = 0; c < C::COUTL; ++c) {
                 const double a = warp_sum((double)s1[c]), b = warp_sum((double)s2[c]);
@@ -515,6 +548,134 @@
                     atomicAdd(&stats[((long)view * C::COUT + co0 + c) * 2 + 1], b);
                 }
             }
+        }
+    } else if constexpr (BNA != 0) {
+        constexpr int P = C::P, TPO = C::BNA_TPO, SEG = C::BNA_SEG, W2 = C::WIN / 2, HW2 = (C::HIN / 2) * W2, NIT = C::BNA_IT;
+        float4* cst_s = reinterpret_cast<float4*>(smem + C::BNA_OFF);
+        float* seg_s = reinterpret_cast<float*>(smem + C::BNA_OFF + C::CIN * 16);
+        const int t = threadIdx.x - 32 * (EPI_END + 1);
+        const int o = t / TPO, s0 = t - o * TPO;
+        const float inv_cnt = 1.0f / ((float)bna.n_per_view * (float)C::HIN * (float)C::WIN);
+        float acc[8];
+#pragma unroll
+        for (int j = 0; j < 8; ++j) acc[j] = 0.f;
+        int cur_view = -1;
+        for (int i = i0; i < i1; ++i) {
+            const int k = i - i0, slot = k % C::SLOTS, use = k / C::SLOTS;
+            const int n = view * n_per_view + i / C::BANDS, band = i % C::BANDS;
+            const int bv = n / bna.n_per_view;
+            if (bv != cur_view) {
+                asm volatile("bar.sync 3, 128;" ::: "memory");
+                if (t < C::CIN) {
+                    const int c = bv * C::CIN + t;
+                    const float a = __ldg(bna.scale + c), b = __ldg(bna.shift + c);
+                    const float is = __ldg(bna.invstd + c), nm = -__ldg(bna.mean + c) * is;
+                    const float k1 = (float)bna.sums[(size_t)c * 2] * inv_cnt, k2 = (float)bna.sums[(size_t)c * 2 + 1] * inv_cnt;
+                    cst_s[t] = make_float4(a, b, -a * is * k2, -a * (k1 + nm * k2));
+                }
+                asm volatile("bar.sync 3, 128;" ::: "memory");
+                cur_view = bv;
+            }
+            const int y0 = band * C::HB - C::PAD;
+            const int wy_lo = y0 > 0 ? y0 / 2 : 0;
+            const int wy_hi = (y0 + C::HPB) / 2 < C::HIN / 2 ? (y0 + C::HPB) / 2 : C::HIN / 2;
+            const int nw = (wy_hi - wy_lo) * W2;
+            const int own_lo = C::BANDS == 1 ? 0 : band * (C::HB / 2), own_hi = C::BANDS == 1 ? C::HIN / 2 : (band + 1) * (C::HB / 2);
+            [[maybe_unused]] uint4 g8[BNA == 1 ? NIT : 1];
+            [[maybe_unused]] float g32[BNA == 2 ? NIT : 1][8];
+#pragma unroll
+            for (int it = 0; it < NIT; ++it) {
+                const int s = s0 + it * TPO;
+                if (s < nw) {
+                    const int wy = wy_lo + s / W2, wx = s % W2;
+                    if constexpr (BNA == 1) {
+                        g8[it] = __ldg(reinterpret_cast<const uint4*>(bna.dp) + ((long)n * P + o) * HW2 + wy * W2 + wx);
+                    } else {
+                        const float* gp = reinterpret_cast<const float*>(bna.dp) + ((long)n * C::CIN + o * 8) * HW2 + wy * W2 + wx;
+#pragma unroll
+                        for (int j = 0; j < 8; ++j) g32[it][j] = __ldg(gp + (long)j * HW2);
+                    }
+                }
+            }
+            mbar_wait(full_bar(slot), use & 1);
+            uint8_t* plane = img_s + slot * C::SLOT_BYTES + o * C::PLANE_BYTES;
+#pragma unroll
+            for (int it = 0; it < NIT; ++it) {
+                const int s = s0 + it * TPO;
+                if (s < nw) {
+                    const int wy = wy_lo + s / W2, wx = s % W2;
+                    const int xp = 2 * wx + C::PAD;
+                    uint4* p00 = reinterpret_cast<uint4*>(plane + (xp % C::XPH) * C::PHASE_BYTES) + (2 * wy - y0) * C::WQ + xp / C::XPH;
+                    uint4* p01 = C::XPH == 1 ? p00 + 1 : reinterpret_cast<uint4*>(reinterpret_cast<uint8_t*>(p00) + C::PHASE_BYTES);
+                    uint4* pw[4] = {p00, p01, p00 + C::WQ, p01 + C::WQ};
+                    float w[4][8], g[8];
+#pragma unroll
+                    for (int q = 0; q < 4; ++q) {
+                        const uint4 r = *pw[q];
+                        const __half2* h = reinterpret_cast<const __half2*>(&r);
+#pragma unroll
+                        for (int e = 0; e < 4; ++e) {
+                            const float2 v = __half22float2(h[e]);
+                            w[q][2 * e] = v.x;
+                            w[q][2 * e + 1] = v.y;
+                        }
+                    }
+                    if constexpr (BNA == 1) {
+                        const uint4 u = g8[it];
+                        const uint32_t gw[4] = {u.x, u.y, u.z, u.w};
+#pragma unroll
+                        for (int e = 0; e < 4; ++e) {
+                            g[2 * e] = __uint_as_float(gw[e] << 16);
+                            g[2 * e + 1] = __uint_as_float(gw[e] & 0xFFFF0000u);
+                        }
+                    } else {
+#pragma unroll
+                        for (int j = 0; j < 8; ++j) g[j] = g32[it][j];
+                    }
+                    const bool own = wy >= own_lo && wy < own_hi;
+#pragma unroll
+                    for (int j = 0; j < 8; ++j) {
+                        const float4 cj = cst_s[o * 8 + j];
+                        float m;
+                        const int kk = argmax4_first(fmaf(cj.x, w[0][j], cj.y), fmaf(cj.x, w[1][j], cj.y), fmaf(cj.x, w[2][j], cj.y),
+                                                     fmaf(cj.x, w[3][j], cj.y), m);
+                        const float gj = (m > 0.f) ? g[j] : 0.f;
+                        const float ag = cj.x * gj;
+#pragma unroll
+                        for (int q = 0; q < 4; ++q) {
+                            w[q][j] = fmaf(cj.z, w[q][j], cj.w) + ((q == kk) ? ag : 0.f);
+                            if (own) acc[j] += w[q][j];
+                        }
+                    }
+                    uint4 d[4];
+#pragma unroll
+                    for (int q = 0; q < 4; ++q) {
+                        d[q] = make_uint4(pack_bf16(w[q][0], w[q][1]), pack_bf16(w[q][2], w[q][3]), pack_bf16(w[q][4], w[q][5]), pack_bf16(w[q][6], w[q][7]));
+                        *pw[q] = d[q];
+                    }
+                    if (own) {
+                        uint4* dst = bna.dz + (((long)n * P + o) * C::HIN + 2 * wy) * C::WIN + 2 * wx;
+                        st_global_256(dst, d[0], d[1]);
+                        st_global_256(dst + C::WIN, d[2], d[3]);
+                    }
+                }
+            }
+            fence_proxy_async_smem();
+            mbar_arrive(ready_bar(slot));
+        }
+#pragma unroll
+        for (int j = 0; j < 8; ++j) {
+            float v = acc[j];
+#pragma unroll
+            for (int dd = SEG / 2; dd > 0; dd >>= 1) v += __shfl_xor_sync(0xffffffffu, v, dd);
+            if (lane % SEG == 0) seg_s[(t / SEG) * 8 + j] = v;
+        }
+        asm volatile("bar.sync 3, 128;" ::: "memory");
+        if (t < C::CIN && bna.dbsum != nullptr) {
+            const int oc = t / 8, j = t % 8;
+            double v = 0.0;
+            for (int sg = oc * TPO / SEG; sg < (oc + 1) * TPO / SEG; ++sg) v += (double)seg_s[sg * 8 + j];
+            atomicAdd(&bna.dbsum[t], v);
         }
     }
     tc_fence_before_sync();
@@ -632,6 +793,52 @@
 }
 
 template <class C>
+int conv_tc_tmaps(const void* x, int N, TMaps* tm) {
+    constexpr uint64_t WT = C::L0 ? C::WQ : C::WIN;
+    for (int r = 0; r < C::XPL; ++r) {
+        const uint64_t dims[4] = {8, WT / C::XPL, (uint64_t)C::HIN, (uint64_t)N * C::P};
+        const uint64_t strides[3] = {16 * (uint64_t)C::XPL, WT * 16, WT * C::HIN * 16};
+        const uint32_t box[4] = {8, (uint32_t)C::WQ, (uint32_t)C::HPB, (uint32_t)C::PC};
+        int rc = encode_tmap_bf16_4d(&tm->m[r], reinterpret_cast<const uint8_t*>(x) + 16 * r, dims, strides, box);
+        if (rc) return rc;
+    }
+    for (int r = C::XPL; r < 4; ++r) tm->m[r] = tm->m[0];
+    return 0;
+}
+
+template <class C>
+int launch_conv_tc_bnapply(const void* z, const void* wprep, void* dx, const BnaArgs& bna, int dp_fmt, int N, cudaStream_t st) {
+    if constexpr (!C::BNA_OK) {
+        set_error("conv_tc_dgrad_bnapply: this geometry has no fused BatchNorm-backward apply");
+        return -5;
+    } else {
+        static bool configured = false;
+        if (!configured) {
+            cudaError_t e = cudaFuncSetAttribute(conv_tc_kernel<C, false, false, 1>, cudaFuncAttributeMaxDynamicSharedMemorySize, C::SMEM_BNA);
+            if (e == cudaSuccess) e = cudaFuncSetAttribute(conv_tc_kernel<C, false, false, 2>, cudaFuncAttributeMaxDynamicSharedMemorySize, C::SMEM_BNA);
+            if (e != cudaSuccess) {
+                set_error("conv_tc_dgrad_bnapply: cannot set %d bytes of shared memory: %s", C::SMEM_BNA, cudaGetErrorString(e));
+                return (int)e;
+            }
+            configured = true;
+        }
+        TMaps tm;
+        int rc = conv_tc_tmaps<C>(z, N, &tm);
+        if (rc) return rc;
+        int G = sm_count() * C::CTAS;
+        const long items = (long)N * C::BANDS;
+        if (G > items) G = (int)items;
+        if (G < 1) G = 1;
+        const uint4* wp = reinterpret_cast<const uint4*>(wprep);
+        if (dp_fmt == 1)
+            conv_tc_kernel<C, false, false, 1><<<dim3(G, 1, 1), C::THREADS + 128, C::SMEM_BNA, st>>>(tm, wp, nullptr, dx, nullptr, N, 1, nullptr, nullptr, nullptr, bna);
+        else
+            conv_tc_kernel<C, false, false, 2><<<dim3(G, 1, 1), C::THREADS + 128, C::SMEM_BNA, st>>>(tm, wp, nullptr, dx, nullptr, N, 1, nullptr, nullptr, nullptr, bna);
+        return launch_status("conv_tc_kernel<bnapply>");
+    }
+}
+
+template <class C>
 int launch_conv_tc(const void* x, const void* wprep, const float* bias, void* out, double* stats, int N, int n_per_view, int out_bf16,
                    cudaStream_t st, void* pool_out = nullptr, const float* gamma = nullptr, const float* beta2 = nullptr) {
     if (pool_out != nullptr && beta2 == nullptr && !C::POOL_OK) {
@@ -651,15 +858,8 @@
         configured = true;
     }
     TMaps tm;
-    constexpr uint64_t WT = C::L0 ? C::WQ : C::WIN;
-    for (int r = 0; r < C::XPL; ++r) {
-        const uint64_t dims[4] = {8, WT / C::XPL, (uint64_t)C::HIN, (uint64_t)N * C::P};
-        const uint64_t strides[3] = {16 * (uint64_t)C::XPL, WT * 16, WT * C::HIN * 16};
-        const uint32_t box[4] = {8, (uint32_t)C::WQ, (uint32_t)C::HPB, (uint32_t)C::PC};
-        int rc = encode_tmap_bf16_4d(&tm.m[r], reinterpret_cast<const uint8_t*>(x) + 16 * r, dims, strides, box);
-        if (rc) return rc;
-    }
-    for (int r = C::XPL; r < 4; ++r) tm.m[r] = tm.m[0];
+    int rc = conv_tc_tmaps<C>(x, N, &tm);
+    if (rc) return rc;
     const int views = N / n_per_view;
     int G = sm_count() * C::CTAS / (views * C::NSPLIT);
     if (G < 1) G = 1;
@@ -1824,4 +2024,38 @@
     return -4;
 }
 
-}
+int b200_conv_tc_dgrad_bnapply_supported(int Cin, int Cout, int H, int W, int K, int pad) {
+#define TC_HAS(CFG) if (Cin == CFG::CIN && Cout == CFG::COUT && H == CFG::HIN && W == CFG::WIN && K == CFG::KS && pad == CFG::PAD) return CFG::BNA_OK ? 1 : 0;
+    TC_HAS(CfgA1d) TC_HAS(CfgA2d) TC_HAS(CfgA3d) TC_HAS(CfgI1d)
+#undef TC_HAS
+    return 0;
+}
+
+int b200_conv_tc_dgrad_bnapply(const void* z8, const void* dp, const float* scale, const float* shift, const float* mean, const float* invstd,
+                               const double* sums, const void* wprep_flip, void* dx_act8, void* dz8, double* dbsum, int N, int n_per_view,
+                               int Cin, int Cout, int H, int W, int K, int pad, int dp_fmt, void* stream) {
+    B200_REQUIRE(z8 && dp && scale && shift && mean && invstd && sums && wprep_flip && dx_act8 && dz8, -1, "conv_tc_dgrad_bnapply: null pointer");
+    B200_REQUIRE(N > 0 && n_per_view > 0 && N % n_per_view == 0, -2, "conv_tc_dgrad_bnapply: N=%d must be a multiple of n_per_view=%d", N, n_per_view);
+    B200_REQUIRE(dp_fmt == 0 || dp_fmt == 1, -2, "conv_tc_dgrad_bnapply: dp_fmt must be 0 (fp32 NCHW) or 1 (bf16 act8)");
+    B200_REQUIRE((((uintptr_t)z8 | (uintptr_t)wprep_flip | (uintptr_t)dx_act8) & 15) == 0 && ((uintptr_t)dz8 & 31) == 0 && ((uintptr_t)dp & 15) == 0, -3,
+                 "conv_tc_dgrad_bnapply: pointers must be 16-byte aligned (dz: 32-byte)");
+    BnaArgs a;
+    a.dp = dp;
+    a.scale = scale;
+    a.shift = shift;
+    a.mean = mean;
+    a.invstd = invstd;
+    a.sums = sums;
+    a.dz = reinterpret_cast<uint4*>(dz8);
+    a.dbsum = dbsum;
+    a.n_per_view = n_per_view;
+    cudaStream_t st = as_stream(stream);
+#define TC_RUN(CFG) if (Cin == CFG::CIN && Cout == CFG::COUT && H == CFG::HIN && W == CFG::WIN && K == CFG::KS && pad == CFG::PAD) \
+        return launch_conv_tc_bnapply<CFG>(z8, wprep_flip, dx_act8, a, dp_fmt == 1 ? 1 : 2, N, st);
+    TC_RUN(CfgA1d) TC_RUN(CfgA2d) TC_RUN(CfgA3d) TC_RUN(CfgI1d)
+#undef TC_RUN
+    set_error("conv_tc_dgrad_bnapply: unsupported geometry Cin=%d Cout=%d H=%d W=%d K=%d pad=%d", Cin, Cout, H, W, K, pad);
+    return -4;
+}
+
+}
diff --git a/multimodal_ssl_avmnist_b200/engine.py b/multimodal_ssl_avmnist_b200/engine.py
--- a/multimodal_ssl_avmnist_b200/engine.py
+++ b/multimodal_ssl_avmnist_b200/engine.py
@@ -162,7 +162,7 @@
                  n_global_views=2, n_local_views=4, momentum=0.996, center_momentum=0.9, student_temperature=0.1,
                  teacher_temperature=0.04, learning_rate=1e-4, weight_decay=1e-6, dropout=0.3, fusion_dropout=0.3, alpha=1.0,
                  cosine_loss_alpha=0.0, augment_values=None, seed=0, device=None, process_group=None, data_parallel=None,
-                 precision="bf16", fused_pool=True, fused_bnstat=False, stream_priorities=False):
+                 precision="bf16", fused_pool=True, fused_bnstat=False, fused_bwd_apply=True, stream_priorities=False):
         if not torch.cuda.is_available():
             raise ops._lib.B200Error("DinoStepEngine needs a CUDA device: the hot path has no CPU fallback")
         ops._lib.load()
@@ -261,6 +261,11 @@
                              ops.conv_tc_dgrad_bnstat_supported(co, ci, hw + 2 * pad - k + 1, hw + 2 * pad - k + 1, k, k - 1 - pad)
                              for li, (conv, bn, ci, co, hw, k, pad) in enumerate(layers)]
                        for mod, layers in (("img", self.img_layers), ("aud", self.aud_layers))}
+        self.fused_bwd_apply = bool(fused_bwd_apply) and kind == "multi_central"
+        self.bnapply = {mod: [self.fused_bwd_apply and li > 0 and bool(self.tc[mod][li]) and not self.bnstat[mod][li] and
+                              ops.conv_tc_dgrad_bnapply_supported(co, ci, hw + 2 * pad - k + 1, hw + 2 * pad - k + 1, k, k - 1 - pad)
+                              for li, (conv, bn, ci, co, hw, k, pad) in enumerate(layers)]
+                        for mod, layers in (("img", self.img_layers), ("aud", self.aud_layers))}
         self._tcw = {}
         self._prep_desc = {}
         for mod, layers in (("img", self.img_layers), ("aud", self.aud_layers)):
@@ -814,6 +819,13 @@
     def _layers(self, mod):
         return self.img_layers if mod == "img" else self.aud_layers
 
+    def _dgrad_out(self, w, mod, li, d_p, N):
+        conv, bn, ci, co, hw, k, pad = self._layers(mod)[li]
+        nxt = w[f"{mod}.dp_a"] if d_p.data_ptr() != w[f"{mod}.dp_a"].data_ptr() else w[f"{mod}.dp_b"]
+        if self.tc[mod][li - 1]:
+            return nxt.view(torch.bfloat16)[:N * ci * hw * hw].view(N, ci // 8, hw, hw, 8)
+        return nxt[:N * ci * hw * hw].view(N, ci, hw, hw)
+
     def _conv_stack_bwd(self, w, mod, layers, x, d_top, N, B):
         S, G = self.S, self.G
         d_p = d_top
@@ -839,12 +851,17 @@
                 if par in busy:
                     main.wait_event(busy.pop(par))
                 fused = ci == 1
+                bna = self.bnapply[mod][li]
                 if not fused:
                     dz = w[f"{mod}.dz8" if par == 0 else f"{mod}.dz8b"][:z.numel()].view_as(z)
                 p_out = w[f"s.{mod}.p8{li}"] if f"s.{mod}.p8{li}" in w else w[f"s.{mod}.p{li}"]
                 if not (li + 1 < len(layers) and self.bnstat[mod][li + 1]):
                     ops.bn_pool8_bwd_reduce_p(p_out, d_p, S["enc." + bn + ".weight"], S["enc." + bn + ".bias"], sums, B)
-                if not fused:
+                if bna:
+                    d_in = self._dgrad_out(w, mod, li, d_p, N)
+                    ops.conv_tc_dgrad_bnapply(z, d_p, self._tcw[("flip", mod, li)], d_in, dz, sc, sh, mu, inv, sums, B, k, k - 1 - pad,
+                                              dbsum=w[f"{mod}.dbsum"][li])
+                elif not fused:
                     ops.bn_relu_pool8_bwd_apply(z, d_p, sc, sh, mu, inv, sums, dz, B, dbsum=w[f"{mod}.dbsum"][li])
             else:
                 dz = w[f"{mod}.dz"][:z.numel()].view_as(z)
@@ -885,19 +902,19 @@
                 xin = x if li == 0 else w[f"s.{mod}.p{li - 1}"]
                 ops.conv_bwd_weight(xin.view(N, ci, hw, hw), dz, G["enc." + conv + ".weight"], G["enc." + conv + ".bias"], w[f"{mod}.wg_work"], pad)
             if li > 0:
-                nxt = w[f"{mod}.dp_a"] if d_p.data_ptr() != w[f"{mod}.dp_a"].data_ptr() else w[f"{mod}.dp_b"]
                 if tc:
-                    if self.tc[mod][li - 1]:
-                        d_in = nxt.view(BF)[:N * ci * hw * hw].view(N, ci // 8, hw, hw, 8)
-                    else:
-                        d_in = nxt[:N * ci * hw * hw].view(N, ci, hw, hw)
-                    if self.bnstat[mod][li]:
+                    if self.bnapply[mod][li]:
+                        pass
+                    elif self.bnstat[mod][li]:
+                        d_in = self._dgrad_out(w, mod, li, d_p, N)
                         lbn = layers[li - 1][1]
                         ops.conv_tc_dgrad_bnstat(dz, self._tcw[("flip", mod, li)], d_in, w[f"s.{mod}.p8{li - 1}"], S["enc." + lbn + ".weight"],
                                                  S["enc." + lbn + ".bias"], w[f"s.{mod}.sums{li - 1}"], B, k, k - 1 - pad)
                     else:
+                        d_in = self._dgrad_out(w, mod, li, d_p, N)
                         ops.conv_tc(dz, self._tcw[("flip", mod, li)], None, d_in, None, N, ci, k, k - 1 - pad)
                 else:
+                    nxt = w[f"{mod}.dp_a"] if d_p.data_ptr() != w[f"{mod}.dp_a"].data_ptr() else w[f"{mod}.dp_b"]
                     d_in = nxt[:N * ci * hw * hw].view(N, ci, hw, hw)
                     ops.conv_bwd_data(dz, S["enc." + conv + ".weight"], d_in, pad)
                 d_p = d_in
diff --git a/multimodal_ssl_avmnist_b200/ops.py b/multimodal_ssl_avmnist_b200/ops.py
--- a/multimodal_ssl_avmnist_b200/ops.py
+++ b/multimodal_ssl_avmnist_b200/ops.py
@@ -293,6 +293,19 @@
     Cout = dx8.shape[1] * 8
     _lib.check(_lib_().b200_conv_tc_dgrad_bnstat(_ptr(dz8, BF16), _ptr(wprep_flip), _ptr(dx8, BF16), _ptr(p8, BF16), _ptr(gamma, F32), _ptr(beta, F32),
                                                  _ptr(sums, F64), N, n_per_view, P * 8, Cout, H, W, K, pad, _stream()), "conv_tc_dgrad_bnstat")
+
+
+def conv_tc_dgrad_bnapply_supported(Cin, Cout, H, W, K, pad):
+    return bool(_lib_().b200_conv_tc_dgrad_bnapply_supported(Cin, Cout, H, W, K, pad))
+
+
+def conv_tc_dgrad_bnapply(z8, dp, wprep_flip, dx8, dz8, scale, shift, mean, invstd, sums, n_per_view, K, pad, dbsum=None):
+    N, P, H, W, _ = z8.shape
+    Cout = dx8.shape[1] * 8
+    _lib.check(_lib_().b200_conv_tc_dgrad_bnapply(_ptr(z8, torch.float16), _ptr(dp), _ptr(scale, F32), _ptr(shift, F32), _ptr(mean, F32),
+                                                  _ptr(invstd, F32), _ptr(sums, F64), _ptr(wprep_flip), _ptr(dx8, BF16), _ptr(dz8, BF16),
+                                                  _ptr(dbsum, F64) if dbsum is not None else None, N, n_per_view, P * 8, Cout, H, W, K, pad,
+                                                  _fmt(dp), _stream()), "conv_tc_dgrad_bnapply")
 
 
 def bn_relu_apply8(e8, scale, shift, out, n_per_view):
@@ -589,7 +602,7 @@
 
 
 _LAUNCHES = {"gate_grad": 2, "ntxent_fwd_bwd": 5, "conv_tc_wgrad_l0_fused": 3, "conv_tc_wgrad": 2, "conv_bwd_weight": 3, "linear_bwd_weight": 3, "infonce_fwd_bwd": 9}
-_NOT_KERNELS = {"conv_tc_wgrad_variant", "gate_grad_work_floats", "knn_predict", "conv_tc_pool_supported", "conv_tc_dgrad_bnstat_supported", "quad8_width", "ntxent_work_floats", "conv_tc_wgrad_l0_fused_work_floats", "conv_tc_wgrad_work_floats", "conv_tc_supported", "conv_tc_weight_bytes", "dino_loss_parts", "infonce_work_floats", "conv_supported", "conv_bwd_weight_work_floats", "launch_count", "start_profile", "stop_profile"}
+_NOT_KERNELS = {"conv_tc_wgrad_variant", "gate_grad_work_floats", "knn_predict", "conv_tc_pool_supported", "conv_tc_dgrad_bnstat_supported", "conv_tc_dgrad_bnapply_supported", "quad8_width", "ntxent_work_floats", "conv_tc_wgrad_l0_fused_work_floats", "conv_tc_wgrad_work_floats", "conv_tc_supported", "conv_tc_weight_bytes", "dino_loss_parts", "infonce_work_floats", "conv_supported", "conv_bwd_weight_work_floats", "launch_count", "start_profile", "stop_profile"}
 LAUNCH_COUNT = 0
 _PROFILE = None
 
```

Result: slower. 132,500 (median of 6 runs) (-2.0%).
